# JuanJoZP/cfd-hemodynamic

Hardware: AMD Instinct MI355X
Metric: time-steps/sec, dfg_1 ~1M DOF (stabilized_schur) (higher is better)
Workload: dtype f64 (fp32 only in the AMG matrix values of the flexible preconditioner and in a read-only copy of the Krylov basis that Gram-Schmidt reads in solves of >= 20 iterations)

## Files before the change

### cfd_hemodynamic_amd/_lib.py

```python
from __future__ import annotations

import ctypes as C
import os
import subprocess

import numpy as np

_HERE = os.path.dirname(os.path.abspath(__file__))
_SO = os.path.join(_HERE, "libcfdh.so")
_LIB = None

dp = C.POINTER(C.c_double)
ip = C.POINTER(C.c_int32)
lp = C.POINTER(C.c_int64)


class Options(C.Structure):
    _fields_ = [
        ("snes_rtol", C.c_double), ("snes_atol", C.c_double), ("snes_stol", C.c_double), ("snes_max_it", C.c_int32),
        ("ksp_rtol", C.c_double), ("ksp_atol", C.c_double), ("ksp_max_it", C.c_int32), ("ksp_restart", C.c_int32),
        ("cheb_degree", C.c_int32), ("cheb_ratio", C.c_double), ("schur_full", C.c_int32),
        ("amg_smooth_degree", C.c_int32), ("amg_smooth_ratio", C.c_double), ("amg_theta", C.c_double),
        ("amg_max_coarse", C.c_int32), ("pc_refresh", C.c_int32), ("remove_p_mean", C.c_int32), ("verbose", C.c_int32),
        ("pc_type", C.c_int32), ("cc_smooth_degree", C.c_int32), ("ksp_guess", C.c_int32),
# ... 73 lines not shown
    L.cfdh_update_dirichlet.argtypes = [vp, C.c_int, C.c_int64, ip, dp]
    L.cfdh_set_state.argtypes = [vp, dp, dp, dp, dp]
    L.cfdh_get_solution.argtypes = [vp, dp, dp]
    L.cfdh_set_time_scheme.argtypes = [vp, C.c_double, C.c_double, C.c_double, C.c_double]
    L.cfdh_set_previous2.argtypes = [vp, dp]
    L.cfdh_get_previous2.argtypes = [vp, dp]
    L.cfdh_shift_history.argtypes = [vp]
    L.cfdh_wall_shear_stress.argtypes = [vp, dp]
    L.cfdh_set_boundary_terms.argtypes = [vp, C.c_int, C.c_int, C.c_double]
    L.cfdh_set_formulation.argtypes = [vp, C.c_int]
    L.cfdh_set_pressure_boundaries.argtypes = [vp, C.c_int, ip, dp, C.c_double]
    L.cfdh_set_pressure_boundaries_ex.argtypes = [vp, C.c_int, ip, dp, C.c_double, C.POINTER(C.c_uint8), dp]
    L.cfdh_get_residual.argtypes = [vp, dp, dp]
    L.cfdh_get_previous.argtypes = [vp, dp, dp]
    L.cfdh_advance.argtypes = [vp]
    L.cfdh_advance_field.argtypes = [vp, C.c_int]
    L.cfdh_assemble.argtypes = [vp, C.c_int]
    L.cfdh_get_csr.argtypes = [vp, lp, ip, ip, dp]
    L.cfdh_spmv.argtypes = [vp, dp, dp]
    L.cfdh_solve_step.argtypes = [vp, C.POINTER(Stats)]
    L.cfdh_functional.argtypes = [vp, C.c_int, C.c_int, dp]
    L.cfdh_set_halo.argtypes = [vp, C.c_int, ip, lp, ip, lp, ip]
    L.cfdh_set_global_pressure_space.argtypes = [vp, C.c_int64, C.c_int64, ip, dp, ip, C.c_int64, ip]
    L.cfdh_comm_unique_id.argtypes = [C.c_void_p]
    L.cfdh_comm_init.argtypes = [vp, C.c_void_p, C.c_int, C.c_int]
    L.cfdh_comm_set_callbacks.argtypes = [vp, ALLREDUCE_FN, EXCHANGE_FN, C.c_void_p, C.c_int, C.c_int]
    L.cfdh_profile_enable.argtypes = [vp, C.c_int]
    L.cfdh_profile_get.argtypes = [vp, C.c_int, dp, lp]
    L.cfdh_profile_reset.argtypes = [vp]
    L.cfdh_info.argtypes = [vp, C.c_int]
    L.cfdh_info.restype = C.c_int64
    L.cfdh_set_schur_pcd.argtypes = [vp, C.c_int, C.c_int, C.c_int]
    L.cfdh_set_ksp_forcing.argtypes = [vp, C.c_int, C.c_double, C.c_double, C.c_double, C.c_double, C.c_double]
    L.cfdh_get_newton_history.argtypes = [vp, ip, dp, dp, ip, dp]
    L.cfdh_get_pcd_operator.argtypes = [vp, lp, ip, ip, dp, dp]
    L.cfdh_apply_preconditioner.argtypes = [vp, dp, dp]
    L.cfdh_apply_operator.argtypes = [vp, dp, dp, dp]
    L.cfdh_get_amg_operator.argtypes = [vp, C.c_int, C.c_int, C.c_int, lp, lp, lp, ip, ip, dp]
    L.cfdh_get_amg_vectors.argtypes = [vp, C.c_int, C.c_int, C.c_int, lp, dp]
    L.cfdh_krylov_vec_op.argtypes = [vp, C.c_int, C.c_int, C.c_int, C.c_int, dp, dp, dp, dp, dp, C.c_double, C.c_int, dp, dp,
                                     C.POINTER(C.c_float), ip, dp, dp, dp]
    L.cfdh_create_ipcs.argtypes = [C.POINTER(vp), C.c_int, C.c_int, C.c_int64, C.c_int64, C.c_int64, ip, dp, C.c_int64, ip, ip, ip]
    L.cfdh_ipcs_set_form.argtypes = [vp, C.c_double, C.c_double]
    L.cfdh_ipcs_set_tolerances.argtypes = [vp, dp, C.c_double, ip]
    L.cfdh_ipcs_step.argtypes = [vp, C.POINTER(IpcsStats)]
    L.cfdh_ipcs_get_operator.argtypes = [vp, C.c_int, lp, ip, ip, dp]
    L.cfdh_ipcs_get_intermediate.argtypes = [vp, C.c_int, dp]
    L.cfdh_ipcs_apply_pressure_pc.argtypes = [vp, dp, dp]
    L.cfdh_ipcs_krylov_solve.argtypes = [vp, C.c_int, dp, dp, C.c_double, C.c_double, C.c_int, dp, C.POINTER(IpcsStats), dp]
    L.cfdh_wall_stats_reset.argtypes = [vp]
    L.cfdh_wall_stats_accumulate.argtypes = [vp, C.c_double]
    L.cfdh_wall_stats_get.argtypes = [vp, C.c_int, lp, dp]
    _LIB = L
    return L


def _dp(a):
    return None if a is None else a.ctypes.data_as(dp)


def _ip(a):
    return None if a is None else a.ctypes.data_as(ip)


def _lp(a):
    return None if a is None else a.ctypes.data_as(lp)


class CfdhError(RuntimeError):
    pass


def _raise(code, msg):
    if code == -1:
        raise ValueError(msg)
    raise CfdhError(msg)


FORM_CONVECTIVE, FORM_ROTATIONAL = 0, 1
PC_SELFP, PC_CAHOUET_CHABARD, PC_PCD = 0, 1, 2
AMG_HIER_A, AMG_HIER_P, AMG_HIER_H = 0, 1, 2
AMG_HIER_PG, AMG_HIER_DL0 = 3, 4
AMG_OP_A, AMG_OP_P, AMG_OP_G, AMG_OP_SB, AMG_OP_SC, AMG_OP_PT = 0, 1, 2, 3, 4, 5
(AMG_VEC_DINV, AMG_VEC_WDINV, AMG_VEC_AGG, AMG_VEC_COARSE_INV, AMG_VEC_D, AMG_VEC_LAMBDA, AMG_VEC_CC_SCALARS, AMG_VEC_CC_ML,
 AMG_VEC_CC_PBC, AMG_VEC_SPGEMM_ROWS, AMG_VEC_SHAPE, AMG_VEC_ORDER, AMG_VEC_A00_LMAX, AMG_VEC_A00_DINV, AMG_VEC_DL0_SHAPE) = range(15)
IP_RHO, IP_RHO_OLD, IP_ALPHA, IP_OMEGA, IP_BETA, IP_RZ, IP_TOL2, IP_BN2, IP_RN2, IP_DONE, IP_ITS, IP_BAD = range(12)
IP_NSCAL = 16

(KVOP_DOT, KVOP_NORM2, KVOP_NORM2_PAIR, KVOP_NORM2_TRIPLE, KVOP_NORMINF_DIFF, KVOP_SUB_MEAN, KVOP_NORM_SCALE_INV, KVOP_MULTIDOT,
 KVOP_MULTIDOT32, KVOP_GRAM, KVOP_MULTIAXPY, KVOP_LINCOMB, KVOP_LINCOMB_KEEP, KVOP_GS_UPDATE_NORMALIZE, KVOP_GS_UPDATE32, KVOP_STORE32,
 KVOP_GUESS, KVOP_AXPY, KVOP_WAXPY, KVOP_SCALE, KVOP_SCALE_TO, KVOP_PMULT) = range(22)
KVOP_FLAG_OPTION, KVOP_FLAG_RING = 1, 2
EW_DEFAULTS = (0.3, 0.9, 1.0, (1.0 + 5.0 ** 0.5) / 2.0, 0.1)
WALL_TAWSS, WALL_OSI, WALL_RRT, WALL_MEAN, WALL_PEAK, WALL_TOTALS = range(6)
INFO_WALL_STATS_COUNT = 90


class Context:

    def __init__(self, x, cells, facet_cells, facet_local, facet_marker, nv_owned=None, device=0, etype=0):
        L = lib()
        self.L = L
        x = np.asarray(x, dtype=np.float64)
        cells = np.asarray(cells)
        self.etype = int(etype)
        self.dim = (3 if x.shape[1] >= 3 and cells.shape[1] in (8, 10) or (self.etype == 3 and cells.shape[1] == 4) else 2) if self.etype \
            else cells.shape[1] - 1
        if self.dim not in (2, 3) or x.shape[1] < self.dim:
            raise ValueError("cells must be triangles [nc,3] or tetrahedra [nc,4] with matching coordinates")
        nodes = {(1, 2): 6, (2, 2): 4, (3, 2): 3, (1, 3): 10, (2, 3): 8, (3, 3): 4}
        if self.etype and cells.shape[1] != nodes[(self.etype, self.dim)]:
            raise ValueError("element type %d needs %d nodes per cell for gdim %d" % (self.etype, nodes[(self.etype, self.dim)], self.dim))
        self.x = np.ascontiguousarray(x[:, : self.dim]).copy()
        self.cells = np.ascontiguousarray(cells, dtype=np.int32)
        self.nv = len(self.x)
        self.nvo = self.nv if nv_owned is None else int(nv_owned)
        fc = np.ascontiguousarray(facet_cells, dtype=np.int32)
        fl = np.ascontiguousarray(facet_local, dtype=np.int32)
        fm = np.ascontiguousarray(facet_marker, dtype=np.int32)
        h = C.c_void_p()
        if self.etype:
            if self.nvo != self.nv:
                rc = L.cfdh_create_elem_part(C.byref(h), int(device), self.dim, self.etype, self.nv, self.nvo, len(self.cells), _ip(self.cells),
                                             _dp(self.x), len(fc), _ip(fc), _ip(fl), _ip(fm))
            else:
                rc = L.cfdh_create_elem(C.byref(h), int(device), self.dim, self.etype, self.nv, len(self.cells), _ip(self.cells), _dp(self.x),
                                        len(fc), _ip(fc), _ip(fl), _ip(fm))
        else:
            rc = L.cfdh_create(C.byref(h), int(device), self.dim, self.nv, self.nvo, len(self.cells), _ip(self.cells), _dp(self.x),
                               len(fc), _ip(fc), _ip(fl), _ip(fm))
        if rc != 0:
            _raise(rc, "cfdh_create failed: " + L.cfdh_last_error(None).decode())
        self.h = h
        self._cb = None

    def close(self):
        if getattr(self, "h", None):
            self.L.cfdh_destroy(self.h)
            self.h = None

    def __del__(self):
        try:
            self.close()
        except Exception:
            pass

    def _chk(self, rc):
        if rc != 0:
            _raise(rc, self.L.cfdh_last_error(self.h).decode())

    def set_params(self, dt, rho, mu, mu_facet=None, f=(0.0, 0.0)):
        ff = np.zeros(3)
        f = np.atleast_1d(np.asarray(f, dtype=np.float64))[:3]
        ff[: len(f)] = f
        self._chk(self.L.cfdh_set_params(self.h, dt, rho, mu, mu if mu_facet is None else mu_facet, _dp(ff)))

    def default_options(self):
        o = Options()
        self.L.cfdh_default_options(C.byref(o))
        return o

    def set_options(self, o):
        self._chk(self.L.cfdh_set_options(self.h, C.byref(o)))

    def clear_dirichlet(self):
        self._chk(self.L.cfdh_clear_dirichlet(self.h))
# ... 379 lines not shown
```

### cfd_hemodynamic_amd/csrc/cfdh_amg_apply.hip

```cpp
#include <hip/hip_runtime.h>

#include "cfdh_internal.hpp"
#include "cfdh_wave.hpp"

struct d3 { double x, y, z; };
__device__ __forceinline__ d3 vzero(const d3 *) { return d3{0.0, 0.0, 0.0}; }
__device__ __forceinline__ d3 vfma(double a, d3 x, d3 acc) { return d3{acc.x + a * x.x, acc.y + a * x.y, acc.z + a * x.z}; }
__device__ __forceinline__ d3 vsub(d3 a, d3 b) { return d3{a.x - b.x, a.y - b.y, a.z - b.z}; }
__device__ __forceinline__ d3 vadd(d3 a, d3 b) { return d3{a.x + b.x, a.y + b.y, a.z + b.z}; }
__device__ __forceinline__ d3 vscale(double a, d3 x) { return d3{a * x.x, a * x.y, a * x.z}; }
__device__ __forceinline__ d3 g8(d3 v) { return d3{group8_sum(v.x), group8_sum(v.y), group8_sum(v.z)}; }
__device__ __forceinline__ d3 wsum(d3 v) { return d3{wave_sum(v.x), wave_sum(v.y), wave_sum(v.z)}; }
__device__ __forceinline__ double vzero(const double *) { return 0.0; }
__device__ __forceinline__ double2 vzero(const double2 *) { return make_double2(0.0, 0.0); }
__device__ __forceinline__ double vfma(double a, double x, double acc) { return acc + a * x; }
__device__ __forceinline__ double2 vfma(double a, double2 x, double2 acc) { return make_double2(acc.x + a * x.x, acc.y + a * x.y); }
__device__ __forceinline__ double vsub(double a, double b) { return a - b; }
__device__ __forceinline__ double2 vsub(double2 a, double2 b) { return make_double2(a.x - b.x, a.y - b.y); }
__device__ __forceinline__ double vadd(double a, double b) { return a + b; }
__device__ __forceinline__ double2 vadd(double2 a, double2 b) { return make_double2(a.x + b.x, a.y + b.y); }
__device__ __forceinline__ double vscale(double a, double x) { return a * x; }
__device__ __forceinline__ double2 vscale(double a, double2 x) { return make_double2(a * x.x, a * x.y); }
__device__ __forceinline__ double g8(double v) { return group8_sum(v); }
__device__ __forceinline__ double2 g8(double2 v) { return make_double2(group8_sum(v.x), group8_sum(v.y)); }
__device__ __forceinline__ double wsum(double v) { return wave_sum(v); }
__device__ __forceinline__ double2 wsum(double2 v) { return make_double2(wave_sum(v.x), wave_sum(v.y)); }

template <int MAXW, typename T>
__device__ __forceinline__ T sell_row_dot(const int *__restrict__ sp, const int *__restrict__ sc, const float *__restrict__ sv,
                                          const T *__restrict__ x, int sl, int lane, T a) {
  sl = __builtin_amdgcn_readfirstlane(sl);
  const int p0 = sp[sl], w = (sp[sl + 1] - p0) >> 6;
  int cidx[MAXW];
  float cval[MAXW];
#pragma unroll
  for (int k = 0; k < MAXW; k++)
    if (k < w) { const int p = p0 + k * 64 + lane; cidx[k] = NTLOAD(sc + p); cval[k] = NTLOAD(sv + p); }
  T g[MAXW];
#pragma unroll
  for (int k = 0; k < MAXW; k++)
    if (k < w) g[k] = x[cidx[k]];
#pragma unroll
  for (int k = 0; k < MAXW; k++)
    if (k < w) a = vfma((double)cval[k], g[k], a);
  for (int k = MAXW; k < w; k++) { const int p = p0 + k * 64 + lane; a = vfma((double)sv[p], x[sc[p]], a); }
  return a;
}

template <int MODE, typename T>
__global__ __launch_bounds__(TPB) void csr_spmv_kernel(int n, const int *__restrict__ rowptr, const int *__restrict__ col,
                                                       const double *__restrict__ val, const T *__restrict__ x,
                                                       T *__restrict__ y, const T *__restrict__ b) {
  const int gid = blockIdx.x * TPB + threadIdx.x;
  const int row = gid >> 3, l = gid & 7;
  T a = vzero((const T *)nullptr);
  if (row < n) {
    const int ks = rowptr[row], ke = rowptr[row + 1];
    for (int k = ks + l; k < ke; k += 8) a = vfma(val[k], x[col[k]], a);
  }
  a = g8(a);
  if (row < n && l == 0) {
    if (MODE == 0) y[row] = a;
    else if (MODE == 1) y[row] = vsub(b[row], a);
    else if (MODE == 2) y[row] = vadd(y[row], a);
    else y[row] = vadd(b[row], a);
  }
}

template <typename T>
static int csr_spmv_t(cfdh_ctx *c, const CsrDev &A, const T *x, T *y, int mode, const T *b) {
  const long long nthreads = 8ll * A.n;
  dim3 grid((unsigned)((nthreads + TPB - 1) / TPB)), block(TPB);
  if (mode == 0) hipLaunchKernelGGL((csr_spmv_kernel<0, T>), grid, block, 0, c->stream, A.n, A.rowptr.p, A.col.p, A.val.p, x, y, b);
  else if (mode == 1) hipLaunchKernelGGL((csr_spmv_kernel<1, T>), grid, block, 0, c->stream, A.n, A.rowptr.p, A.col.p, A.val.p, x, y, b);
  else if (mode == 2) hipLaunchKernelGGL((csr_spmv_kernel<2, T>), grid, block, 0, c->stream, A.n, A.rowptr.p, A.col.p, A.val.p, x, y, b);
  else hipLaunchKernelGGL((csr_spmv_kernel<3, T>), grid, block, 0, c->stream, A.n, A.rowptr.p, A.col.p, A.val.p, x, y, b);
  HIPCHK(c, hipGetLastError());
  return 0;
}
int k_csr_spmv(cfdh_ctx *c, const CsrDev &A, const double *x, double *y, int mode, const double *b) {
  return csr_spmv_t<double>(c, A, x, y, mode, b);
}
int k_csr_spmv_ncol(cfdh_ctx *c, const CsrDev &A, const double *x, double *y, int mode, const double *b, int ncol) {
  if (ncol == 2) return csr_spmv_t<double2>(c, A, (const double2 *)x, (double2 *)y, mode, (const double2 *)b);
  if (ncol == 3) return csr_spmv_t<d3>(c, A, (const d3 *)x, (d3 *)y, mode, (const d3 *)b);
  return csr_spmv_t<double>(c, A, x, y, mode, b);
}

template <int MODE, bool LAST>
__global__ __launch_bounds__(TPB) void cheb_csr_step_kernel(int n, const int *__restrict__ rowptr, const int *__restrict__ col,
                                                            const double *__restrict__ val, const double *__restrict__ dinv,
                                                            const double *__restrict__ rin, double *__restrict__ rout,
                                                            const double *__restrict__ dold, double *__restrict__ dnew,
                                                            double *__restrict__ x, double c1, double c2, double itheta) {
  const int gid = blockIdx.x * TPB + threadIdx.x;
  const int row = gid >> 3, l = gid & 7;
  double a = 0;
  if (row < n) {
    const int ks = rowptr[row], ke = rowptr[row + 1];
    for (int k = ks + l; k < ke; k += 8) {
      const int j = col[k];
      a += val[k] * (MODE == 1 ? dinv[j] * rin[j] * itheta : dold[j]);
    }
  }
  a = group8_sum(a);
  if (row < n && l == 0) {
    const double di = dinv[row], ri = rin[row];
    const double dd = (MODE == 1) ? di * ri * itheta : dold[row];
    const double r = ri - a;
    const double dn = c1 * dd + c2 * di * r;
    if (!LAST) { rout[row] = r; dnew[row] = dn; }
    if (MODE == 0) x[row] += dn;
    else if (MODE == 1) x[row] = dd + dn;
    else x[row] += dd + dn;
  }
}

__global__ __launch_bounds__(TPB) void csr_resid_init_kernel(int n, const int *__restrict__ rowptr, const int *__restrict__ col,
                                                             const double *__restrict__ val, const double *__restrict__ dinv,
                                                             const double *__restrict__ b, const double *__restrict__ x,
                                                             double *__restrict__ r, double *__restrict__ d0, double itheta) {
  const int gid = blockIdx.x * TPB + threadIdx.x;
  const int row = gid >> 3, l = gid & 7;
  double a = 0;
  if (row < n) {
    const int ks = rowptr[row], ke = rowptr[row + 1];
    for (int k = ks + l; k < ke; k += 8) a += val[k] * x[col[k]];
  }
  a = group8_sum(a);
  if (row < n && l == 0) {
    const double rr = b[row] - a;
    r[row] = rr;
    d0[row] = dinv[row] * rr * itheta;
  }
}

static int level_cheb(cfdh_ctx *c, AmgLevel *L, const double *b, double *x, bool zero_guess, int deg, bool prof) {
  const int n = L->n;
  const double theta = 0.5 * (L->lmax + L->lmin), delta = 0.5 * (L->lmax - L->lmin), sigma = theta / delta;
  double rho = 1.0 / sigma;
  double *dold = L->d0.p, *dnew = L->d1.p, *r = L->r.p;
  const double *rin = b;
  const double itheta = 1.0 / theta;
  const long long nthreads = 8ll * n;
  dim3 grid((unsigned)((nthreads + TPB - 1) / TPB)), block(TPB);
  const int *rp = L->A.rowptr.p, *cl = L->A.col.p;
  const double *vl = L->A.val.p, *di = L->dinv.p;
  if (deg == 1) {
    if (!zero_guess) { CHK(k_csr_spmv(c, L->A, x, r, 1, b)); rin = r; }
    return k_cheb_init(c, n, di, rin, dold, x, itheta, zero_guess ? 0 : 1, nullptr);
  }
  if (!zero_guess) {
    hipLaunchKernelGGL(csr_resid_init_kernel, grid, block, 0, c->stream, n, rp, cl, vl, di, b, x, r, dold, itheta);
    rin = r;
  }
  for (int k = 1; k < deg; k++) {
    const double rho_new = 1.0 / (2.0 * sigma - rho);
    const double c1 = rho_new * rho, c2 = 2.0 * rho_new / delta;
    const bool last = (k == deg - 1);
    const int mode = (k == 1) ? (zero_guess ? 1 : 2) : 0;
    if (prof) prof_begin(c, 4);
#define LAUNCH_STEP(M, LST) hipLaunchKernelGGL((cheb_csr_step_kernel<M, LST>), grid, block, 0, c->stream, n, rp, cl, vl, di, rin, r, dold, dnew, x, c1, c2, itheta)
    if (mode == 1) { if (last) LAUNCH_STEP(1, true); else LAUNCH_STEP(1, false); }
    else if (mode == 2) { if (last) LAUNCH_STEP(2, true); else LAUNCH_STEP(2, false); }
    else { if (last) LAUNCH_STEP(0, true); else LAUNCH_STEP(0, false); }
#undef LAUNCH_STEP
    if (prof) prof_end(c, 4);
    rin = r;
    std::swap(dold, dnew);
    rho = rho_new;
  }
  HIPCHK(c, hipGetLastError());
  return 0;
}
int k_level_smooth(cfdh_ctx *c, AmgLevel *L, const double *b, double *x, int degree) { return level_cheb(c, L, b, x, true, degree, false); }

__global__ __launch_bounds__(TPB) void sell_cheb2_scale_kernel(int n, const int *__restrict__ sptr, const int *__restrict__ scol,
                                                               const float *__restrict__ svalw, const double *__restrict__ wdinv,
                                                               const double *__restrict__ dinv, const double *__restrict__ b,
                                                               double *__restrict__ x, const double *__restrict__ ml,
                                                               double *__restrict__ y, double c1, double c2) {
  const int row = blockIdx.x * TPB + threadIdx.x;
  if (row >= n) return;
  const int sl = row >> 6, lane = row & 63;
  const int p0 = sptr[sl], w = (sptr[sl + 1] - p0) >> 6;
  (void)p0; (void)w;
  const double a = sell_row_dot<10, double>(sptr, scol, svalw, b, sl, lane, 0.0);
  const double bi = b[row];
  const double dd = wdinv[row] * bi;
  const double xv = dd + (c1 * dd + c2 * dinv[row] * (bi - a));
  x[row] = xv;
  y[row] = ml[row] * xv;
}
bool k_cc_cheb2_scale(cfdh_ctx *c, AmgLevel *L, const double *b, double *x, const double *ml, double *y) {
  const int n = L->n;
  if (!(cfdh_cheb2_sell(L->A.nnz, n) && L->A.has_sell_weighted())) return false;
  const double theta = 0.5 * (L->lmax + L->lmin), delta = 0.5 * (L->lmax - L->lmin), sigma = theta / delta;
  const double rho = 1.0 / sigma, rho_new = 1.0 / (2.0 * sigma - rho);
  const double c1 = rho_new * rho, c2 = 2.0 * rho_new / delta;
  hipLaunchKernelGGL(sell_cheb2_scale_kernel, dim3((n + TPB - 1) / TPB), dim3(TPB), 0, c->stream, n, L->A.sptr.p, L->A.scol.p,
                     L->A.svalw.p, L->wdinv.p, L->dinv.p, b, x, ml, y, c1, c2);
  return hipGetLastError() == hipSuccess;
}

template <typename T>
__global__ __launch_bounds__(64) void dense_mv_kernel(int n, const double *__restrict__ Minv, const T *__restrict__ b,
                                                      T *__restrict__ y) {
  const int row = blockIdx.x, l = threadIdx.x;
  T a = vzero((const T *)nullptr);
  for (int k = l; k < n; k += 64) a = vfma(Minv[(size_t)row * n + k], b[k], a);
  a = wsum(a);
  if (l == 0) y[row] = a;
}

template <typename T>
__global__ __launch_bounds__(TPB) void jacobi_pre_kernel(int n, const int *__restrict__ rowptr, const int *__restrict__ col,
                                                         const double *__restrict__ val, const double *__restrict__ wdinv,
                                                         const T *__restrict__ b, T *__restrict__ xa, T *__restrict__ r) {
  const int gid = blockIdx.x * TPB + threadIdx.x;
  const int row = gid >> 3, l = gid & 7;
  T a = vzero((const T *)nullptr);
  if (row < n) {
    const int ks = rowptr[row], ke = rowptr[row + 1];
    for (int k = ks + l; k < ke; k += 8) {
      const int j = col[k];
      a = vfma(val[k] * wdinv[j], b[j], a);
    }
  }
  a = g8(a);
  if (row < n && l == 0) {
    const T bi = b[row];
    xa[row] = vscale(wdinv[row], bi);
    r[row] = vsub(bi, a);
  }
}
template <typename T>
__global__ __launch_bounds__(TPB) void jacobi_post_kernel(int n, const int *__restrict__ rowptr, const int *__restrict__ col,
                                                          const double *__restrict__ val, const double *__restrict__ wdinv,
                                                          const T *__restrict__ b, const T *__restrict__ xin,
                                                          T *__restrict__ xout) {
  const int gid = blockIdx.x * TPB + threadIdx.x;
  const int row = gid >> 3, l = gid & 7;
  T a = vzero((const T *)nullptr);
  if (row < n) {
    const int ks = rowptr[row], ke = rowptr[row + 1];
    for (int k = ks + l; k < ke; k += 8) a = vfma(val[k], xin[col[k]], a);
  }
  a = g8(a);
  if (row < n && l == 0) {
    xout[row] = vadd(xin[row], vscale(wdinv[row], vsub(b[row], a)));
  }
}

template <int MODE, typename T>
__global__ __launch_bounds__(TPB) void sell_spmv_kernel(int n, const int *__restrict__ sptr, const int *__restrict__ scol,
                                                        const float *__restrict__ sval, const T *__restrict__ x,
                                                        T *__restrict__ y, const T *__restrict__ b) {
  const int row = blockIdx.x * TPB + threadIdx.x;
  if (row >= n) return;
  const int sl = row >> 6, lane = row & 63;
  const int p0 = sptr[sl], w = (sptr[sl + 1] - p0) >> 6;
  T a = vzero((const T *)nullptr);
#pragma unroll 4
  for (int k = 0; k < w; k++) {
    const int p = p0 + k * 64 + lane;
    a = vfma((double)sval[p], x[scol[p]], a);
  }
  if (MODE == 0) y[row] = a;
  else if (MODE == 1) y[row] = vsub(b[row], a);
  else if (MODE == 2) y[row] = vadd(y[row], a);
  else y[row] = vadd(b[row], a);
}
template <typename T>
__global__ __launch_bounds__(TPB) void sell_jacobi_pre_kernel(int n, const int *__restrict__ sptr, const int *__restrict__ scol,
                                                              const float *__restrict__ svalw, const double *__restrict__ wdinv,
                                                              const T *__restrict__ b, T *__restrict__ xa, T *__restrict__ r) {
  const int row = blockIdx.x * TPB + threadIdx.x;
  if (row >= n) return;
  const int sl = row >> 6, lane = row & 63;
  const int p0 = sptr[sl], w = (sptr[sl + 1] - p0) >> 6;
  T a = vzero((const T *)nullptr);
#pragma unroll 4
  for (int k = 0; k < w; k++) {
    const int p = p0 + k * 64 + lane;
// ... 20 lines not shown
  }
  xout[row] = vadd(xin[row], vscale(wdinv[row], vsub(b[row], a)));
}

template <typename T>
static void launch_jacobi_pre(cfdh_ctx *c, const CsrDev &A, bool sell, int n, const double *wdinv, const T *b, T *xa, T *r) {
  dim3 block(TPB), gridS((unsigned)((n + TPB - 1) / TPB)), gridC((unsigned)((8ll * n + TPB - 1) / TPB));
  if (cfdh_pre_takes_sell(A, sell))
    hipLaunchKernelGGL((sell_jacobi_pre_kernel<T>), gridS, block, 0, c->stream, n, A.sptr.p, A.scol.p, A.svalw.p, wdinv, b, xa, r);
  else
    hipLaunchKernelGGL((jacobi_pre_kernel<T>), gridC, block, 0, c->stream, n, A.rowptr.p, A.col.p, A.val.p, wdinv, b, xa, r);
}
template <typename T>
static void launch_jacobi_post(cfdh_ctx *c, const CsrDev &A, bool sell, int n, const double *wdinv, const T *b, const T *x1, T *x) {
  dim3 block(TPB), gridS((unsigned)((n + TPB - 1) / TPB)), gridC((unsigned)((8ll * n + TPB - 1) / TPB));
  if (cfdh_post_takes_sell(A, sell))
    hipLaunchKernelGGL((sell_jacobi_post_kernel<T>), gridS, block, 0, c->stream, n, A.sptr.p, A.scol.p, A.sval.p, wdinv, b, x1, x);
  else
    hipLaunchKernelGGL((jacobi_post_kernel<T>), gridC, block, 0, c->stream, n, A.rowptr.p, A.col.p, A.val.p, wdinv, b, x1, x);
}
template <typename T>
static void launch_prolong_add(cfdh_ctx *c, const CsrDev &P, bool sell, int n, const T *x, T *y, const T *b) {
  dim3 block(TPB), gridS((unsigned)((n + TPB - 1) / TPB)), gridC((unsigned)((8ll * n + TPB - 1) / TPB));
  if (cfdh_prolong_takes_sell(P, sell))
    hipLaunchKernelGGL((sell_spmv_kernel<3, T>), gridS, block, 0, c->stream, n, P.sptr.p, P.scol.p, P.sval.p, x, y, b);
  else
    hipLaunchKernelGGL((csr_spmv_kernel<3, T>), gridC, block, 0, c->stream, n, P.rowptr.p, P.col.p, P.val.p, x, y, b);
}

template <typename T>
static int amg_cycle_jacobi(cfdh_ctx *c, AmgHier &H, size_t lev, const T *b, T *x, int prof) {
  AmgLevel *L = H.lev[lev];
  if (lev + 1 == H.lev.size()) {
    if (H.coarse_n > 0) {
      hipLaunchKernelGGL((dense_mv_kernel<T>), dim3(H.coarse_n), dim3(64), 0, c->stream, H.coarse_n, H.coarse_inv.p, b, x);
    } else {
      const int n = L->n;
      T *xa = (T *)L->d0.p, *r = (T *)L->r.p;
      launch_jacobi_pre<T>(c, L->A, false, n, L->wdinv.p, b, xa, r);
      launch_jacobi_post<T>(c, L->A, false, n, L->wdinv.p, b, (const T *)xa, x);
    }
    HIPCHK(c, hipGetLastError());
    return 0;
  }
  AmgLevel *N = H.lev[lev + 1];
  const int n = L->n;
  const bool sell = cfdh_sweep_sell(L->A.nnz, n);
  T *xa = (T *)L->d0.p, *x1 = (T *)L->d1.p, *r = (T *)L->r.p;
  if (prof && lev == 0) prof_begin(c, prof);
  launch_jacobi_pre<T>(c, L->A, sell, n, L->wdinv.p, b, xa, r);
  if (prof && lev == 0) prof_end(c, prof);
  CHK(csr_spmv_t<T>(c, L->R, r, (T *)N->b.p, 0, (const T *)nullptr));
  CHK(amg_cycle_jacobi<T>(c, H, lev + 1, (const T *)N->b.p, (T *)N->x.p, prof));
  launch_prolong_add<T>(c, L->P, sell, n, (const T *)N->x.p, x1, (const T *)xa);
  HIPCHK(c, hipGetLastError());
  if (prof && lev == 0) prof_begin(c, prof);
  launch_jacobi_post<T>(c, L->A, sell, n, L->wdinv.p, b, (const T *)x1, x);
  if (prof && lev == 0) prof_end(c, prof);
  HIPCHK(c, hipGetLastError());
  return 0;
}

template <int LPR>
__device__ __forceinline__ double lpr_sum(double v) {
  v = group8_sum(v);
  if (LPR >= 16) v += dpp_shuffle<0x140>(v);
  if (LPR >= 32) v += __shfl_xor(v, 16);
  if (LPR >= 64) v += __shfl_xor(v, 32);
  return v;
}
template <int LPR> __device__ __forceinline__ double lsum(double v) { return lpr_sum<LPR>(v); }
template <int LPR> __device__ __forceinline__ double2 lsum(double2 v) { return make_double2(lpr_sum<LPR>(v.x), lpr_sum<LPR>(v.y)); }
template <int LPR> __device__ __forceinline__ d3 lsum(d3 v) { return d3{lpr_sum<LPR>(v.x), lpr_sum<LPR>(v.y), lpr_sum<LPR>(v.z)}; }

__device__ __forceinline__ double epi_apply(double acc, int row, double alpha, double beta, const double *zH, const double *r, const unsigned char *pbc) {
  return (pbc[row] & 1) ? r[row] : alpha * acc + beta * zH[row];
}
__device__ __forceinline__ double2 epi_apply(double2 acc, int, double, double, const double *, const double *, const unsigned char *) { return acc; }
__device__ __forceinline__ double epi_value(double acc, unsigned flag, double alpha, double beta, double zh, double r) { return (flag & 1u) ? r : alpha * acc + beta * zh; }
__device__ __forceinline__ double2 epi_value(double2 acc, unsigned, double, double, double, double) { return acc; }
__device__ __forceinline__ d3 epi_apply(d3 acc, int, double, double, const double *, const double *, const unsigned char *) { return acc; }
__device__ __forceinline__ d3 epi_value(d3 acc, unsigned, double, double, double, double) { return acc; }

template <int LPR, typename VT, typename T>
__global__ __launch_bounds__(TPB) void fused_down_kernel(int n, const int *__restrict__ rowptr, const int *__restrict__ col,
                                                         const VT *__restrict__ val, const T *__restrict__ x, T *__restrict__ y) {
  const int gid = blockIdx.x * TPB + threadIdx.x;
  const int row = gid / LPR, l = gid % LPR;
  T a = vzero((const T *)nullptr);
  if (row < n) {
    const int ks = rowptr[row], ke = rowptr[row + 1];
    int cidx[4];
    VT cval[4];
#pragma unroll
    for (int q = 0; q < 4; q++) { const int k = ks + l + q * LPR; if (k < ke) { cidx[q] = col[k]; cval[q] = val[k]; } }
    T g[4];
#pragma unroll
    for (int q = 0; q < 4; q++) { const int k = ks + l + q * LPR; if (k < ke) g[q] = x[cidx[q]]; }
#pragma unroll
    for (int q = 0; q < 4; q++) { const int k = ks + l + q * LPR; if (k < ke) a = vfma((double)cval[q], g[q], a); }
    for (int k = ks + l + 4 * LPR; k < ke; k += LPR) a = vfma((double)val[k], x[col[k]], a);
  }
  a = lsum<LPR>(a);
  if (row < n && l == 0) y[row] = a;
}
template <typename T>
__global__ __launch_bounds__(TPB) void fused_up_csr_kernel(int n, const int *__restrict__ rpB, const int *__restrict__ clB,
                                                           const double *__restrict__ vlB, const T *__restrict__ b,
                                                           const int *__restrict__ rpC, const int *__restrict__ clC,
                                                           const double *__restrict__ vlC, const T *__restrict__ xc,
                                                           T *__restrict__ x, double ea, double eb, const double *__restrict__ ezH,
                                                           const double *__restrict__ er, const unsigned char *__restrict__ epbc) {
  const int gid = blockIdx.x * TPB + threadIdx.x;
  const int row = gid >> 3, l = gid & 7;
  T a = vzero((const T *)nullptr);
  if (row < n) {
    const int kb = rpB[row] + l, keB = rpB[row + 1];
    int kc = 0, keC = 0;
    if (rpC) { kc = rpC[row] + l; keC = rpC[row + 1]; }
    int cb[2], cc[2];
    double vb[2], vc[2];
#pragma unroll
    for (int q = 0; q < 2; q++) {
      if (kb + 8 * q < keB) { cb[q] = clB[kb + 8 * q]; vb[q] = vlB[kb + 8 * q]; }
      if (kc + 8 * q < keC) { cc[q] = clC[kc + 8 * q]; vc[q] = vlC[kc + 8 * q]; }
    }
    T gb[2], gc[2];
#pragma unroll
    for (int q = 0; q < 2; q++) {
      if (kb + 8 * q < keB) gb[q] = b[cb[q]];
      if (kc + 8 * q < keC) gc[q] = xc[cc[q]];
    }
#pragma unroll
    for (int q = 0; q < 2; q++) {
      if (kb + 8 * q < keB) a = vfma(vb[q], gb[q], a);
      if (kc + 8 * q < keC) a = vfma(vc[q], gc[q], a);
    }
    for (int k = kb + 16; k < keB; k += 8) a = vfma(vlB[k], b[clB[k]], a);
    for (int k = kc + 16; k < keC; k += 8) a = vfma(vlC[k], xc[clC[k]], a);
  }
  a = g8(a);
  if (row < n && l == 0) x[row] = epbc ? epi_apply(a, row, ea, eb, ezH, er, epbc) : a;
}
template <typename T, bool WIDE>
__global__ __launch_bounds__(TPB) void fused_up_sell_kernel(int n, const int *__restrict__ spB, const int *__restrict__ scB,
                                                            const float *__restrict__ svB, const T *__restrict__ b,
                                                            const int *__restrict__ spC, const int *__restrict__ scC,
                                                            const float *__restrict__ svC, const T *__restrict__ xc,
                                                            T *__restrict__ x, double ea, double eb, const double *__restrict__ ezH,
                                                            const double *__restrict__ er, const unsigned char *__restrict__ epbc) {
  const int row = blockIdx.x * TPB + threadIdx.x;
  if (row >= n) return;
  const int sl = __builtin_amdgcn_readfirstlane(row >> 6), lane = row & 63;
  T a = vzero((const T *)nullptr);
  double e_zh = 0.0, e_r = 0.0;
  unsigned e_f = 0;
  if (epbc) { e_f = epbc[row]; e_zh = ezH[row]; e_r = er[row]; }
  constexpr int MW = sizeof(T) > 8 ? 8 : 10;
  const int pB = spB[sl], wB = (spB[sl + 1] - pB) >> 6;
  int pC = 0, wC = 0;
  if (spC) { pC = spC[sl]; wC = (spC[sl + 1] - pC) >> 6; }
  const int wmax = wB > wC ? wB : wC;
  for (int k0 = 0; k0 < (WIDE ? wmax : 1); k0 += MW) {
    int cB[MW], cC[MW];
    float vB[MW], vC[MW];
#pragma unroll
    for (int k = 0; k < MW; k++) if (k0 + k < wB) { const int p = pB + (k0 + k) * 64 + lane; cB[k] = NTLOAD(scB + p); vB[k] = NTLOAD(svB + p); }
#pragma unroll
    for (int k = 0; k < MW; k++) if (k0 + k < wC) { const int p = pC + (k0 + k) * 64 + lane; cC[k] = NTLOAD(scC + p); vC[k] = NTLOAD(svC + p); }
    T gB[MW], gC[MW];
#pragma unroll
    for (int k = 0; k < MW; k++) if (k0 + k < wB) gB[k] = b[cB[k]];
#pragma unroll
    for (int k = 0; k < MW; k++) if (k0 + k < wC) gC[k] = xc[cC[k]];
#pragma unroll
    for (int k = 0; k < MW; k++) if (k0 + k < wB) a = vfma((double)vB[k], gB[k], a);
#pragma unroll
    for (int k = 0; k < MW; k++) if (k0 + k < wC) a = vfma((double)vC[k], gC[k], a);
  }
  if (!WIDE) {
    for (int k = MW; k < wB; k++) { const int p = pB + k * 64 + lane; a = vfma((double)svB[p], b[scB[p]], a); }
    for (int k = MW; k < wC; k++) { const int p = pC + k * 64 + lane; a = vfma((double)svC[p], xc[scC[p]], a); }
  }
  x[row] = epbc ? epi_value(a, e_f, ea, eb, e_zh, e_r) : a;
}
template <typename T>
__global__ __launch_bounds__(TPB) void fused_up_dense_kernel(int n, const int *__restrict__ rpB, const int *__restrict__ clB,
                                                             const double *__restrict__ vlB, const T *__restrict__ b,
                                                             const float *__restrict__ D, int nc, const T *__restrict__ bc,
                                                             T *__restrict__ x) {
  const int gid = blockIdx.x * TPB + threadIdx.x;
  const int row = gid >> 6, l = gid & 63;
  T a = vzero((const T *)nullptr);
  if (row < n) {
    for (int k = rpB[row] + l, ke = rpB[row + 1]; k < ke; k += 64) a = vfma(vlB[k], b[clB[k]], a);
    const float *Dr = D + (size_t)row * nc;
    float dv[12];
    T bv[12];
#pragma unroll
    for (int q = 0; q < 12; q++) { const int j = l + 64 * q; if (j < nc) { dv[q] = Dr[j]; bv[q] = bc[j]; } }
#pragma unroll
    for (int q = 0; q < 12; q++) { const int j = l + 64 * q; if (j < nc) a = vfma((double)dv[q], bv[q], a); }
    for (int j = l + 768; j < nc; j += 64) a = vfma((double)Dr[j], bc[j], a);
  }
  a = wsum(a);
  if (row < n && l == 0) x[row] = a;
}

template <typename VT, typename T>
static void launch_down(cfdh_ctx *c, const CsrDev &G, const VT *val, const T *x, T *y) {
  const long long avg = G.n > 0 ? (G.nnz + G.n - 1) / G.n : 1;
  const int lpr = avg > 96 ? 64 : (avg > 48 ? 32 : (avg > 20 ? 16 : 8));
  dim3 block(TPB), grid((unsigned)(((long long)G.n * lpr + TPB - 1) / TPB));
  if (lpr == 64) hipLaunchKernelGGL((fused_down_kernel<64, VT, T>), grid, block, 0, c->stream, G.n, G.rowptr.p, G.col.p, val, x, y);
  else if (lpr == 32) hipLaunchKernelGGL((fused_down_kernel<32, VT, T>), grid, block, 0, c->stream, G.n, G.rowptr.p, G.col.p, val, x, y);
  else if (lpr == 16) hipLaunchKernelGGL((fused_down_kernel<16, VT, T>), grid, block, 0, c->stream, G.n, G.rowptr.p, G.col.p, val, x, y);
  else hipLaunchKernelGGL((fused_down_kernel<8, VT, T>), grid, block, 0, c->stream, G.n, G.rowptr.p, G.col.p, val, x, y);
}

template <typename T>
static int amg_cycle_fused(cfdh_ctx *c, AmgHier &H, const T *b, T *x, int prof, int l0 = 0) {
  const int nl = (int)H.lev.size();
  for (int l = l0; l + 1 < nl; l++) {
    AmgLevel *L = H.lev[l], *N = H.lev[l + 1];
    const T *src = l == l0 ? b : (const T *)L->b.p;
    if (prof && l == 0) prof_begin(c, prof + 4);
    if (L->fine) launch_down<float, T>(c, L->G, L->G.valf.p, src, (T *)N->b.p);
    else launch_down<double, T>(c, L->G, L->G.val.p, src, (T *)N->b.p);
    if (prof && l == 0) prof_end(c, prof + 4);
  }
  int l = nl - 1;
  {
    AmgLevel *L = H.lev[l];
    const T *bl = l == l0 ? b : (const T *)L->b.p;
    T *xl = l == l0 ? x : (T *)L->x.p;
    if (nl - 2 >= l0 && H.lev[nl - 2]->Dn > 0) {
      AmgLevel *U = H.lev[nl - 2];
      const T *bu = nl - 2 == l0 ? b : (const T *)U->b.p;
      T *xu = nl - 2 == l0 ? x : (T *)U->x.p;
      const int un = (nl - 2 == 0 && c->up0_rows > 0 && c->up0_rows < U->n) ? c->up0_rows : U->n;
      hipLaunchKernelGGL((fused_up_dense_kernel<T>), dim3((unsigned)((64ll * un + TPB - 1) / TPB)), dim3(TPB), 0, c->stream, un,
                         U->Sb.rowptr.p, U->Sb.col.p, U->Sb.val.p, bu, U->D.p, U->Dn, bl, xu);
      l = nl - 3;
    } else {
      if (H.coarse_n > 0)
        hipLaunchKernelGGL((dense_mv_kernel<T>), dim3(H.coarse_n), dim3(64), 0, c->stream, H.coarse_n, H.coarse_inv.p, bl, xl);
      else if (L->sell)
        hipLaunchKernelGGL((fused_up_sell_kernel<T, true>), dim3((unsigned)((L->n + TPB - 1) / TPB)), dim3(TPB), 0, c->stream, L->n,
                           L->Sb.sptr.p, L->Sb.scol.p, L->Sb.sval.p, bl, (const int *)nullptr, (const int *)nullptr,
                           (const float *)nullptr, (const T *)nullptr, xl, 0.0, 0.0, (const double *)nullptr, (const double *)nullptr,
                           (const unsigned char *)nullptr);
      else
        hipLaunchKernelGGL((fused_up_csr_kernel<T>), dim3((unsigned)((8ll * L->n + TPB - 1) / TPB)), dim3(TPB), 0, c->stream, L->n,
                           L->Sb.rowptr.p, L->Sb.col.p, L->Sb.val.p, bl, (const int *)nullptr, (const int *)nullptr,
                           (const double *)nullptr, (const T *)nullptr, xl, 0.0, 0.0, (const double *)nullptr, (const double *)nullptr,
                           (const unsigned char *)nullptr);
      l = nl - 2;
    }
  }
  for (; l >= l0; l--) {
    AmgLevel *L = H.lev[l], *N = H.lev[l + 1];
    const T *bl = l == l0 ? b : (const T *)L->b.p;
    T *xl = l == l0 ? x : (T *)L->x.p;
    const bool epi = l == 0 && c->epi.on && sizeof(T) == sizeof(double);
    const double ea = epi ? c->epi.alpha : 0.0, eb = epi ? c->epi.beta : 0.0;
    const double *ezH = epi ? c->epi.zH : nullptr, *er = epi ? c->epi.r : nullptr;
    const unsigned char *epbc = epi ? c->epi.pbc : nullptr;
    if (epi) { xl = (T *)c->epi.out; c->epi.done = true; }
    const int nrow = (l == 0 && c->up0_rows > 0 && c->up0_rows < L->n) ? c->up0_rows : L->n;
    if (prof && l == 0) prof_begin(c, prof);
    if (L->sell && L->Sb.sell_maxw <= 14 && L->Sc.sell_maxw <= 14)
      hipLaunchKernelGGL((fused_up_sell_kernel<T, false>), dim3((unsigned)((nrow + TPB - 1) / TPB)), dim3(TPB), 0, c->stream, nrow,
                         L->Sb.sptr.p, L->Sb.scol.p, L->Sb.sval.p, bl, L->Sc.sptr.p, L->Sc.scol.p, L->Sc.sval.p, (const T *)N->x.p, xl,
                         ea, eb, ezH, er, epbc);
    else if (L->sell)
      hipLaunchKernelGGL((fused_up_sell_kernel<T, true>), dim3((unsigned)((nrow + TPB - 1) / TPB)), dim3(TPB), 0, c->stream, nrow,
                         L->Sb.sptr.p, L->Sb.scol.p, L->Sb.sval.p, bl, L->Sc.sptr.p, L->Sc.scol.p, L->Sc.sval.p, (const T *)N->x.p, xl,
                         ea, eb, ezH, er, epbc);
    else
      hipLaunchKernelGGL((fused_up_csr_kernel<T>), dim3((unsigned)((8ll * nrow + TPB - 1) / TPB)), dim3(TPB), 0, c->stream, nrow,
                         L->Sb.rowptr.p, L->Sb.col.p, L->Sb.val.p, bl, L->Sc.rowptr.p, L->Sc.col.p, L->Sc.val.p, (const T *)N->x.p, xl,
                         ea, eb, ezH, er, epbc);
    if (prof && l == 0) prof_end(c, prof);
  }
  HIPCHK(c, hipGetLastError());
  return 0;
}

static int amg_cycle_cheb(cfdh_ctx *c, AmgHier &H, size_t lev, const double *b, double *x, bool prof) {
  AmgLevel *L = H.lev[lev];
  if (lev + 1 == H.lev.size()) {
    if (H.coarse_n > 0) {
      hipLaunchKernelGGL((dense_mv_kernel<double>), dim3(H.coarse_n), dim3(64), 0, c->stream, H.coarse_n, H.coarse_inv.p, b, x);
      HIPCHK(c, hipGetLastError());
      return 0;
    }
    return level_cheb(c, L, b, x, true, c->opt.amg_smooth_degree > 2 ? c->opt.amg_smooth_degree : 2, false);
  }
  AmgLevel *N = H.lev[lev + 1];
  const int deg = c->opt.amg_smooth_degree;
  CHK(level_cheb(c, L, b, x, true, deg, prof && lev == 0));
  CHK(k_csr_spmv(c, L->A, x, L->r.p, 1, b));
  CHK(k_csr_spmv(c, L->R, L->r.p, N->b.p, 0, nullptr));
  CHK(amg_cycle_cheb(c, H, lev + 1, N->b.p, N->x.p, prof));
  CHK(k_csr_spmv(c, L->P, N->x.p, x, 2, nullptr));
  CHK(level_cheb(c, L, b, x, false, deg, prof && lev == 0));
  return 0;
}

__global__ __launch_bounds__(TPB) void dl0_pack_kernel(int nvo, int nv, int dim, const double *__restrict__ vec, const double *__restrict__ wdinv,
                                                       double *__restrict__ b, double *__restrict__ xa, int ghosts) {
  const int i = blockIdx.x * TPB + threadIdx.x;
  if (i >= nv) return;
  const double v = i < nvo ? vec[(size_t)dim * nvo + i] : (ghosts ? vec[((size_t)dim + 1) * nvo + ((size_t)dim + 1) * (size_t)(i - nvo) + dim] : 0.0);
  b[i] = v;
  xa[i] = wdinv[i] * v;
}
int k_dl0_down(cfdh_ctx *c, const double *halo_vec) {
  cfdh_ctx::DistL0 &d = c->dl0;
  AmgLevel *N = c->hLg.lev[1];
  const int nvo = c->nvo, nv = c->nv;
  if (d.ghost_rhs) hipLaunchKernelGGL(dl0_pack_kernel, dim3((nv + TPB - 1) / TPB), dim3(TPB), 0, c->stream, nvo, nv, c->dim, halo_vec, d.wdinv.p, d.b.p, d.xa.p, 1);
  launch_jacobi_pre<double>(c, d.A, cfdh_dl0_rule_A(c), nvo, d.wdinv.p, (const double *)d.b.p, d.xa.p, d.r.p);
  HIPCHK(c, hipGetLastError());
  return csr_spmv_t<double>(c, d.PT, d.r.p, N->b.p, 0, (const double *)nullptr);
}
int k_dl0_up(cfdh_ctx *c, double *out) {
  cfdh_ctx::DistL0 &d = c->dl0;
  AmgLevel *N = c->hLg.lev[1];
  const int nvo = c->nvo, nv = c->nv;
  if (cfdh_dl0_coarse_fused(c)) CHK(amg_cycle_fused<double>(c, c->hLg, (const double *)N->b.p, N->x.p, 0, 1));
  else CHK(amg_cycle_jacobi<double>(c, c->hLg, 1, (const double *)N->b.p, N->x.p, 0));
  launch_prolong_add<double>(c, d.P, cfdh_dl0_rule_P(c), nv, (const double *)N->x.p, d.x1.p, (const double *)d.xa.p);
  HIPCHK(c, hipGetLastError());
  launch_jacobi_post<double>(c, d.A, cfdh_dl0_rule_A(c), nvo, d.wdinv.p, (const double *)d.b.p, (const double *)d.x1.p, out);
  HIPCHK(c, hipGetLastError());
  return 0;
}

int k_amg_vcycle(cfdh_ctx *c, AmgHier &H, const double *b, double *x) {
  if (!H.valid || H.lev.empty()) return cfdh_fail(c, CFDH_E_STATE, "AMG hierarchy not built");
  const bool prof = (&H == &c->hS) || (&H == &c->hL) || (&H == &c->hLg);
  if (H.ncol == 3) {
    if (H.fused && c->opt.amg_smooth_degree == 1 && H.lev.size() >= 2) return amg_cycle_fused<d3>(c, H, (const d3 *)b, (d3 *)x, 5);
    return amg_cycle_jacobi<d3>(c, H, 0, (const d3 *)b, (d3 *)x, 5);
  }
  if (H.fused && c->opt.amg_smooth_degree == 1 && H.lev.size() >= 2) {
    if (H.ncol == 2) return amg_cycle_fused<double2>(c, H, (const double2 *)b, (double2 *)x, 5);
    return amg_cycle_fused<double>(c, H, b, x, prof ? 4 : 0);
  }
  if (H.ncol == 2) return amg_cycle_jacobi<double2>(c, H, 0, (const double2 *)b, (double2 *)x, 5);
  if (c->opt.amg_smooth_degree == 1) return amg_cycle_jacobi<double>(c, H, 0, b, x, prof ? 4 : 0);
  return amg_cycle_cheb(c, H, 0, b, x, prof);
}

__global__ __launch_bounds__(TPB) void cc_scale_kernel(int n, const double *__restrict__ ml, const double *__restrict__ z, double *__restrict__ y) {
  const int i = blockIdx.x * TPB + threadIdx.x;
  if (i < n) y[i] = ml[i] * z[i];
}
__global__ __launch_bounds__(TPB) void cc_combine_kernel(int n, double alpha, double beta, const double *__restrict__ t,
                                                         const double *__restrict__ z, const double *__restrict__ r,
                                                         const unsigned char *__restrict__ pbc, double *__restrict__ out, double *__restrict__ out2) {
  const int i = blockIdx.x * TPB + threadIdx.x;
  if (i < n) {
    const double v = (pbc[i] & 1) ? r[i] : alpha * t[i] + beta * z[i];
// ... 59 lines not shown
```

### cfd_hemodynamic_amd/csrc/cfdh_api.cpp

```cpp
#include <algorithm>
#include <cmath>
#include <numeric>

#include <dlfcn.h>

#include "cfdh_internal.hpp"
#include "cfdh_ipcs.hpp"

std::string g_cfdh_last_error;

int cfdh_prepare_assembly(cfdh_ctx *c);

#define ENTER(c)                         \
  do {                                   \
    if (!(c)) return CFDH_E_ARG;         \
    (void)hipSetDevice((c)->device);     \
  } while (0)

#define NOT_IPCS(c, name)                                                                                                    \
  do {                                                                                                                       \
    if ((c) && (c)->ipcs) return cfdh_fail((c), CFDH_E_STATE, name ": not available on an incremental pressure-correction context (cfdh_create_ipcs)"); \
  } while (0)
#define NEED_IPCS(c, name)                                                                                         \
  do {                                                                                                             \
    if (!(c)) return CFDH_E_ARG;                                                                                   \
    if (!(c)->ipcs) return cfdh_fail((c), CFDH_E_STATE, name ": the context was not created by cfdh_create_ipcs"); \
    (void)hipSetDevice((c)->device);                                                                               \
  } while (0)

static int ipcs_put(cfdh_ctx *c, dbuf<double> &dst, const double *src) {
  if (!src) return 0;
  c->ipcs->n_field_copies++;
  HIPCHK(c, hipMemcpyAsync(dst.p, src, sizeof(double) * dst.n, hipMemcpyHostToDevice, c->stream));
  HIPCHK(c, hipStreamSynchronize(c->stream));
  return 0;
}
static int ipcs_get(cfdh_ctx *c, const dbuf<double> &src, double *dst) {
  if (!dst) return 0;
  c->ipcs->n_field_copies++;
  HIPCHK(c, hipMemcpyAsync(dst, src.p, sizeof(double) * src.n, hipMemcpyDeviceToHost, c->stream));
  HIPCHK(c, hipStreamSynchronize(c->stream));
  return 0;
}
static int ipcs_copy(cfdh_ctx *c, const dbuf<double> &src, dbuf<double> &dst) {
  HIPCHK(c, hipMemcpyAsync(dst.p, src.p, sizeof(double) * src.n, hipMemcpyDeviceToDevice, c->stream));
  return 0;
}

namespace {
template <class T>
struct HookBuf {
  T *p = nullptr;
  ~HookBuf() { if (p) (void)hipFree(p); }
  int put(cfdh_ctx *c, const T *src, size_t count, size_t filled) {
    HIPCHK(c, hipMalloc((void **)&p, sizeof(T) * count));
    HIPCHK(c, hipMemsetAsync(p, 0, sizeof(T) * count, c->stream));
    if (src && filled) HIPCHK(c, hipMemcpyAsync(p, src, sizeof(T) * filled, hipMemcpyHostToDevice, c->stream));
    return 0;
  }
  int get(cfdh_ctx *c, T *dst, size_t count) const {
    HIPCHK(c, hipMemcpy(dst, p, sizeof(T) * count, hipMemcpyDeviceToHost));
    return 0;
  }
};
}

extern "C" {

int cfdh_abi_version(void) { return CFDH_ABI_VERSION; }

const char *cfdh_last_error(const cfdh_ctx *c) { return c ? c->err.c_str() : g_cfdh_last_error.c_str(); }

int cfdh_default_options(cfdh_options *o) {
  if (!o) return CFDH_E_ARG;
  o->snes_rtol = 1e-8; o->snes_atol = 1e-50; o->snes_stol = 1e-8; o->snes_max_it = 100;
  o->ksp_rtol = 1e-5; o->ksp_atol = 1e-50; o->ksp_max_it = 1000; o->ksp_restart = 200;
  o->cheb_degree = 3; o->cheb_ratio = 10.0; o->schur_full = 2;
  o->amg_smooth_degree = 1; o->amg_smooth_ratio = 8.0; o->amg_theta = -1.0; o->amg_max_coarse = 1000;
  o->pc_refresh = 0; o->remove_p_mean = 1; o->verbose = 0; o->pc_type = 1; o->cc_smooth_degree = 2;
  o->ksp_guess = getenv("CFDH_KSP_GUESS") ? atoi(getenv("CFDH_KSP_GUESS")) : 4;
  return 0;
}

static int create_ctx(cfdh_ctx **out, int device, int gdim, int etype, int64_t nv, int64_t nv_owned, int64_t nc, const int32_t *cells,
                      const double *coords, int64_t nfacets, const int32_t *facet_cells, const int32_t *facet_local,
                      const int32_t *facet_marker) {
  if (!out) return cfdh_fail(nullptr, CFDH_E_ARG, "null output pointer");
  *out = nullptr;
  if (gdim != 2 && gdim != 3) return cfdh_fail(nullptr, CFDH_E_ARG, "gdim must be 2 (P1 triangles) or 3 (P1 tetrahedra)");
  if (etype < 0 || etype > 3) return cfdh_fail(nullptr, CFDH_E_ARG, "unknown element type %d", etype);
  if (!cells || !coords || (nfacets > 0 && (!facet_cells || !facet_local)))
    return cfdh_fail(nullptr, CFDH_E_ARG, "null mesh array");
  int ndev = 0;
  if (hipGetDeviceCount(&ndev) != hipSuccess || ndev <= 0)
    return cfdh_fail(nullptr, CFDH_E_HIP, "no HIP device available: libcfdh has no CPU fallback");
  if (device < 0 || device >= ndev) return cfdh_fail(nullptr, CFDH_E_ARG, "device %d out of range (%d devices)", device, ndev);
  cfdh_ctx *c = new (std::nothrow) cfdh_ctx();
  if (!c) return cfdh_fail(nullptr, CFDH_E_NOMEM, "out of host memory");
  c->device = device;
  cfdh_default_options(&c->opt);
  { const char *e = getenv("CFDH_NO_GRAPH"); c->use_graph = !(e && e[0] == '1'); }
  { const char *e = getenv("CFDH_SOLVE_LEAN"); c->lean = !(e && e[0] == '0'); }
  {
    cfdh_ctx::SolveEnv &v = c->env;
    const char *e;
    if ((e = getenv("CFDH_KRYLOV_FP32"))) v.krylov_fp32 = atoi(e);
    v.guess_check = getenv("CFDH_GUESS_CHECK") != nullptr;
    e = getenv("CFDH_NO_ATTAINABLE_STOP"); v.no_attainable_stop = e && e[0] == '1';
    if ((e = getenv("CFDH_GS_REFINE_FROM"))) v.gs_refine_from = atoi(e);
    if ((e = getenv("CFDH_KSP_LAG"))) v.ksp_lag = atoi(e);
    if ((e = getenv("CFDH_GS_ETA2"))) v.gs_eta2 = atof(e);
    if ((e = getenv("CFDH_L_CYCLES"))) v.l_cycles = atoi(e);
    if ((e = getenv("CFDH_A_CYCLES"))) v.a_cycles = atoi(e);
    e = getenv("CFDH_DL0_COARSE_SWEEPS"); v.dl0_coarse_sweeps = e && e[0] == '1';
  }
  if (c->use_graph && (getenv("ROCP_TOOL_LIBRARIES") || dlsym(RTLD_DEFAULT, "rocprofiler_configure"))) {
    int rt = 0;
    const char *ov = getenv("CFDH_GRAPH_UNDER_PROFILER");
    if (!(ov && ov[0] == '1') && hipRuntimeGetVersion(&rt) == hipSuccess && rt >= 70200000) c->use_graph = false;
  }
  memset(&c->last_stats, 0, sizeof c->last_stats);
  int rc = 0;
  do {
    if (hipSetDevice(device) != hipSuccess) { rc = cfdh_fail(nullptr, CFDH_E_HIP, "hipSetDevice(%d) failed", device); break; }
    if (hipStreamCreateWithFlags(&c->stream, hipStreamNonBlocking) != hipSuccess) { rc = cfdh_fail(nullptr, CFDH_E_HIP, "hipStreamCreate failed"); break; }
    rc = gdim == 3 ? k3_upload_quadrature(c) : k_upload_quadrature(c);
    if (rc) break;
    if (etype != 0) {
      rc = gdim == 3 ? kg3_upload_tables(c) : kg_upload_tables(c);
      if (rc) break;
      rc = gdim == 3 ? cfdh_build_mesh_gen3(c, etype, nv, nv_owned, nc, cells, coords, nfacets, facet_cells, facet_local, facet_marker)
                     : cfdh_build_mesh_gen(c, etype, nv, nv_owned, nc, cells, coords, nfacets, facet_cells, facet_local, facet_marker);
      break;
    }
    rc = gdim == 3 ? cfdh_build_mesh3(c, nv, nv_owned, nc, cells, coords, nfacets, facet_cells, facet_local, facet_marker)
                   : cfdh_build_mesh(c, nv, nv_owned, nc, cells, coords, nfacets, facet_cells, facet_local, facet_marker);
  } while (0);
  if (rc) {
    g_cfdh_last_error = c->err.empty() ? g_cfdh_last_error : c->err;
    cfdh_destroy(c);
    return rc;
  }
  *out = c;
  return 0;
}

int cfdh_create(cfdh_ctx **out, int device, int gdim, int64_t nv, int64_t nv_owned, int64_t nc, const int32_t *cells,
                const double *coords, int64_t nfacets, const int32_t *facet_cells, const int32_t *facet_local,
                const int32_t *facet_marker) {
  return create_ctx(out, device, gdim, CFDH_ELEM_P1, nv, nv_owned, nc, cells, coords, nfacets, facet_cells, facet_local, facet_marker);
}

int cfdh_create_elem(cfdh_ctx **out, int device, int gdim, int elem, int64_t nn, int64_t nc, const int32_t *cells, const double *node_coords,
                     int64_t nfacets, const int32_t *facet_cells, const int32_t *facet_local, const int32_t *facet_marker) {
  return create_ctx(out, device, gdim, elem, nn, nn, nc, cells, node_coords, nfacets, facet_cells, facet_local, facet_marker);
}

int cfdh_create_elem_part(cfdh_ctx **out, int device, int gdim, int elem, int64_t nn, int64_t nn_owned, int64_t nc, const int32_t *cells,
                          const double *node_coords, int64_t nfacets, const int32_t *facet_cells, const int32_t *facet_local, const int32_t *facet_marker) {
  return create_ctx(out, device, gdim, elem, nn, nn_owned, nc, cells, node_coords, nfacets, facet_cells, facet_local, facet_marker);
}

void cfdh_destroy(cfdh_ctx *c) {
  if (!c) return;
  (void)hipSetDevice(c->device);
  if (c->stream) (void)hipStreamSynchronize(c->stream);
  cfdh_ipcs_free(c);
  comm_finalize(c);
  c->hS.clear(); c->hL.clear(); c->hA.clear(); c->hLg.clear();
  for (hipEvent_t e : c->ev_pool) (void)hipEventDestroy(e);
  for (auto &e : c->pc_graphs) for (auto &x : e.exec) if (x) (void)hipGraphExecDestroy(x);
  if (c->h_pinned) (void)hipHostFree(c->h_pinned);
  if (c->h_stage) (void)hipHostFree(c->h_stage);
  if (c->ev_h) (void)hipEventDestroy(c->ev_h);
  if (c->h_big) (void)hipHostFree(c->h_big);
  if (c->h_ring) (void)hipHostFree(c->h_ring);
  for (hipEvent_t e : c->ev_ring) if (e) (void)hipEventDestroy(e);
  hipStream_t s = c->stream;
  delete c;
  if (s) (void)hipStreamDestroy(s);
}

int cfdh_set_params(cfdh_ctx *c, double dt, double rho, double mu, double mu_facet, const double f[3]) {
  ENTER(c);
  if (!(dt > 0) || !(rho > 0) || !(mu > 0)) return cfdh_fail(c, CFDH_E_ARG, "dt, rho, mu must be positive");
// ... 586 lines not shown
      CHK(v_multidot(c, n, dA.p, ld, nvec, dx.p, ds.p, ww, mir_dev)); nd = nm = nvec + (ww ? 1 : 0); break;
    }
    case CFDH_KVOP_MULTIDOT32: CHK(v_multidot32(c, n, dA32.p, ld, nvec, dx.p, ds.p, mir_dev)); nd = nm = nvec + 1; break;
    case CFDH_KVOP_GRAM: CHK(v_gram(c, n, dA.p, ld, nvec, dx.p, ds.p)); nd = 8 * (nvec + 1); break;
    case CFDH_KVOP_MULTIAXPY:
      HIPCHK(c, hipMemcpyAsync(d1.p, dx.p, sizeof(double) * N, hipMemcpyDeviceToDevice, c->stream));
      CHK(v_multiaxpy(c, n, dA.p, ld, nvec, dc.p, d1.p)); break;
    case CFDH_KVOP_LINCOMB:
      HIPCHK(c, hipMemcpyAsync(d1.p, dx.p, sizeof(double) * N, hipMemcpyDeviceToDevice, c->stream));
      CHK(v_lincomb(c, n, dA.p, ld, nvec, dc.p, d1.p)); break;
    case CFDH_KVOP_LINCOMB_KEEP:
      HIPCHK(c, hipMemcpyAsync(d1.p, dx.p, sizeof(double) * N, hipMemcpyDeviceToDevice, c->stream));
      CHK(v_lincomb_keep(c, n, dA.p, ld, nvec, dc.p, d1.p, d2.p)); break;
    case CFDH_KVOP_GS_UPDATE_NORMALIZE: CHK(v_gs_update_normalize(c, n, dA.p, ld, nvec, dc.p, dx.p, d1.p, ds.p)); nd = 1; break;
    case CFDH_KVOP_GS_UPDATE32:
      CHK(v_gs_update32(c, n, dA32.p, ld, nvec, dc.p, dx.p, d1.p, d32.p, ds.p, mir_dev + (nvec + 1))); nd = 1; nm = nvec + 2; break;
    case CFDH_KVOP_STORE32: CHK(v_store32(c, n, dx.p, d32.p)); break;
    case CFDH_KVOP_GUESS: {
      CHK(v_guess_combine(c, n, dA.p, dB.p, ld, nvec, dc.p, dx.p, d1.p, d2.p));
      bool used = false; int rank = 0;
      CHK(v_guess_read(c, nvec, scal_host, &used, &rank, scal_host + 3));
      scal_host[1] = used ? 1.0 : 0.0; scal_host[2] = (double)rank;
      if (flags & 1) CHK(v_scale_inv_lean(c, n, d2.p));
      ns = nm = 3 + nvec;
      HIPCHK(c, hipMemcpyAsync(ds.p, c->red_out.p + RO_LEAN_S2, sizeof(double), hipMemcpyDeviceToDevice, c->stream));
      HIPCHK(c, hipMemcpyAsync(ds.p + 1, c->ky.p, sizeof(double) * nvec, hipMemcpyDeviceToDevice, c->stream));
      nd = 1 + nvec; break;
    }
    case CFDH_KVOP_AXPY:
      HIPCHK(c, hipMemcpyAsync(d1.p, dy.p, sizeof(double) * N, hipMemcpyDeviceToDevice, c->stream));
      CHK(v_axpy(c, n, scalar, dx.p, d1.p)); break;
    case CFDH_KVOP_WAXPY: CHK(v_waxpy(c, n, scalar, dx.p, dy.p, d1.p)); break;
    case CFDH_KVOP_SCALE:
      HIPCHK(c, hipMemcpyAsync(d1.p, dx.p, sizeof(double) * N, hipMemcpyDeviceToDevice, c->stream));
      CHK(v_scale(c, n, scalar, d1.p)); break;
    case CFDH_KVOP_SCALE_TO: CHK(v_scale_to(c, n, scalar, dx.p, d1.p)); break;
    case CFDH_KVOP_PMULT: CHK(v_pointwise_mult(c, n, dx.p, dy.p, d1.p)); break;
  }
  HIPCHK(c, hipStreamSynchronize(c->stream));
  if (nd) HIPCHK(c, hipMemcpy(scal_dev, dev_src, sizeof(double) * nd, hipMemcpyDeviceToHost));
  for (int i = 0; i < nm; i++) scal_mirror[i] = mir_host[i];
  nscal[0] = ns; nscal[1] = nd; nscal[2] = nm;
  if (o1) CHK(d1.get(c, out1, N));
  if (o2) CHK(d2.get(c, out2, N));
  if (o32) CHK(d32.get(c, out32, N));
  return 0;
}

static int amg_pick(cfdh_ctx *c, const char *name, int hier, int level, AmgHier **H, AmgLevel **L) {
  if (!c->pc_valid) return cfdh_fail(c, CFDH_E_STATE, "%s: no preconditioner built yet (cfdh_apply_preconditioner or cfdh_solve_step first)", name);
  *H = nullptr;
  *L = nullptr;
  if (hier == CFDH_AMG_HIER_H) {
    if (c->opt.pc_type != 1 || c->Hlev.n <= 0) return cfdh_fail(c, CFDH_E_STATE, "%s: H exists for pc_type 1 only", name);
    *L = &c->Hlev;
    return 0;
  }
  if (hier == CFDH_AMG_HIER_DL0) {
    if (c->gp_n <= 0 || !c->hLg.valid || !c->dl0.on) return cfdh_fail(c, CFDH_E_STATE, "%s: no distributed finest pressure level on this context", name);
    *H = &c->hLg;
    return 0;
  }
  if (hier != CFDH_AMG_HIER_A && hier != CFDH_AMG_HIER_P && hier != CFDH_AMG_HIER_PG) return cfdh_fail(c, CFDH_E_ARG, "%s: unknown hierarchy %d", name, hier);
  if (hier == CFDH_AMG_HIER_A && c->opt.pc_type == 0) return cfdh_fail(c, CFDH_E_STATE, "%s: pc_type 0 has no velocity hierarchy", name);
  if (hier == CFDH_AMG_HIER_PG && c->gp_n <= 0) return cfdh_fail(c, CFDH_E_STATE, "%s: no replicated pressure space (cfdh_set_global_pressure_space)", name);
  AmgHier *h = hier == CFDH_AMG_HIER_A ? &c->hA : hier == CFDH_AMG_HIER_PG ? &c->hLg : (c->opt.pc_type == 0 ? &c->hS : &c->hL);
  if (!h->valid) return cfdh_fail(c, CFDH_E_STATE, "%s: hierarchy %d is not built", name, hier);
  if (level < 0 || level >= (int)h->lev.size()) return cfdh_fail(c, CFDH_E_ARG, "%s: level %d of %d", name, level, (int)h->lev.size());
  *H = h;
  *L = h->lev[level];
  return 0;
}
static bool amg_local_dim(const cfdh_ctx *c, int n) { return n == (int)c->perm.size() || n == c->nvo; }

int cfdh_get_amg_operator(cfdh_ctx *c, int hier, int level, int which, int64_t *nrow, int64_t *ncol, int64_t *nnz, int32_t *rowptr,
                          int32_t *col, double *vals) {
  NOT_IPCS(c, "cfdh_get_amg_operator");
  if (!c || !nrow || !ncol || !nnz) return CFDH_E_ARG;
  ENTER(c);
  AmgHier *H = nullptr;
  AmgLevel *L = nullptr;
  CHK(amg_pick(c, "cfdh_get_amg_operator", hier, level, &H, &L));
  const bool dl0 = hier == CFDH_AMG_HIER_DL0;
  if (dl0 ? (which != CFDH_AMG_OP_A && which != CFDH_AMG_OP_P && which != CFDH_AMG_OP_PT) : (which < CFDH_AMG_OP_A || which > CFDH_AMG_OP_SC))
    return cfdh_fail(c, CFDH_E_ARG, "cfdh_get_amg_operator: unknown operator %d", which);
  if (!H || dl0) level = 0;
  const CsrDev &M = dl0 ? (which == CFDH_AMG_OP_A ? c->dl0.A : which == CFDH_AMG_OP_P ? c->dl0.P : c->dl0.PT)
                        : which == CFDH_AMG_OP_A ? L->A : which == CFDH_AMG_OP_P ? L->P : which == CFDH_AMG_OP_G ? L->G : which == CFDH_AMG_OP_SB ? L->Sb : L->Sc;
  if (M.n <= 0 || !M.rowptr.p || !M.col.p || !M.val.p)
    return cfdh_fail(c, CFDH_E_STATE, "cfdh_get_amg_operator: operator %d of level %d is not kept in fp64 CSR (P: CFDH_AMG_KEEP=1 before the build)", which, level);
  *nrow = M.n; *ncol = M.m; *nnz = M.nnz;
  if (!rowptr && !col && !vals) return 0;
  if (!rowptr || !col || !vals) return cfdh_fail(c, CFDH_E_ARG, "pass all of rowptr/col/vals or none");
  std::vector<int> rp((size_t)M.n + 1), cl((size_t)M.nnz);
  std::vector<double> vl((size_t)M.nnz);
  HIPCHK(c, hipMemcpyAsync(rp.data(), M.rowptr.p, sizeof(int) * rp.size(), hipMemcpyDeviceToHost, c->stream));
  if (M.nnz > 0) {
    HIPCHK(c, hipMemcpyAsync(cl.data(), M.col.p, sizeof(int) * cl.size(), hipMemcpyDeviceToHost, c->stream));
    HIPCHK(c, hipMemcpyAsync(vl.data(), M.val.p, sizeof(double) * vl.size(), hipMemcpyDeviceToHost, c->stream));
  }
  HIPCHK(c, hipStreamSynchronize(c->stream));
  if (rp[M.n] != M.nnz) return cfdh_fail(c, CFDH_E_STATE, "cfdh_get_amg_operator: rowptr ends at %d, the operator holds %d entries", rp[M.n], M.nnz);
  const bool local0 = level == 0 && hier != CFDH_AMG_HIER_PG;
  const bool rows0 = local0 && which != CFDH_AMG_OP_G && which != CFDH_AMG_OP_PT && amg_local_dim(c, M.n);
  const bool cols0 = local0 && (which == CFDH_AMG_OP_A || which == CFDH_AMG_OP_SB || which == CFDH_AMG_OP_G || which == CFDH_AMG_OP_PT) && amg_local_dim(c, M.m);
  const bool resort = cols0 && which != CFDH_AMG_OP_PT;
  int64_t pos = 0;
  std::vector<std::pair<int, double>> row;
  for (int ru = 0; ru < M.n; ru++) {
    const int r = rows0 ? c->perm[ru] : ru;
    rowptr[ru] = (int32_t)pos;
    row.clear();
    for (int k = rp[r]; k < rp[r + 1]; k++) row.push_back({cols0 ? c->iperm[cl[k]] : cl[k], vl[k]});
    if (resort) std::stable_sort(row.begin(), row.end(), [](const std::pair<int, double> &a, const std::pair<int, double> &b) { return a.first < b.first; });
    for (auto &e : row) { col[pos] = e.first; vals[pos] = e.second; pos++; }
  }
  rowptr[M.n] = (int32_t)pos;
  return 0;
}

int cfdh_get_amg_vectors(cfdh_ctx *c, int hier, int level, int which, int64_t *n, double *out) {
  NOT_IPCS(c, "cfdh_get_amg_vectors");
  if (!c || !n) return CFDH_E_ARG;
  ENTER(c);
  AmgHier *H = nullptr;
  AmgLevel *L = nullptr;
  CHK(amg_pick(c, "cfdh_get_amg_vectors", hier, level, &H, &L));
  const bool dl0 = hier == CFDH_AMG_HIER_DL0;
  if (!H || dl0) level = 0;
  if (dl0 && which != CFDH_AMG_VEC_WDINV && which != CFDH_AMG_VEC_ORDER && which != CFDH_AMG_VEC_DL0_SHAPE)
    return cfdh_fail(c, CFDH_E_ARG, "cfdh_get_amg_vectors: the distributed level has no item %d", which);
  AmgLevel dl0_view;
  if (dl0) { dl0_view.n = c->nv; L = &dl0_view; }
  const bool perm0 = level == 0 && hier != CFDH_AMG_HIER_PG && amg_local_dim(c, L->n);
  auto fetch = [&](const void *src, size_t bytes, void *dst) -> int {
    HIPCHK(c, hipMemcpyAsync(dst, src, bytes, hipMemcpyDeviceToHost, c->stream));
    HIPCHK(c, hipStreamSynchronize(c->stream));
    return 0;
  };
  const int nvo = c->nvo;
  switch (which) {
    case CFDH_AMG_VEC_DINV:
    case CFDH_AMG_VEC_WDINV: {
      const dbuf<double> &v = dl0 ? c->dl0.wdinv : which == CFDH_AMG_VEC_DINV ? L->dinv : L->wdinv;
      if (!v.p || (int)v.n < L->n) return cfdh_fail(c, CFDH_E_STATE, "cfdh_get_amg_vectors: vector %d is not there", which);
      *n = L->n;
      if (!out) return 0;
      std::vector<double> h((size_t)L->n);
      CHK(fetch(v.p, sizeof(double) * h.size(), h.data()));
      for (int i = 0; i < L->n; i++) out[i] = h[perm0 ? c->perm[i] : i];
      return 0;
    }
    case CFDH_AMG_VEC_AGG: {
      if (!L->agg.p || (int)L->agg.n < L->n) return cfdh_fail(c, CFDH_E_STATE, "cfdh_get_amg_vectors: the aggregate ids were not kept (CFDH_AMG_KEEP=1 before the build)");
      *n = L->n;
      if (!out) return 0;
      std::vector<int> h((size_t)L->n);
      CHK(fetch(L->agg.p, sizeof(int) * h.size(), h.data()));
      for (int i = 0; i < L->n; i++) out[i] = (double)h[perm0 ? c->perm[i] : i];
      return 0;
    }
    case CFDH_AMG_VEC_COARSE_INV: {
      if (!H || H->coarse_n <= 0 || !H->coarse_inv.p) return cfdh_fail(c, CFDH_E_STATE, "cfdh_get_amg_vectors: no dense coarsest inverse");
      *n = (int64_t)H->coarse_n * H->coarse_n;
      if (!out) return 0;
      if (H->lev.size() == 1 && hier != CFDH_AMG_HIER_PG && amg_local_dim(c, H->coarse_n)) {
        const size_t m = (size_t)H->coarse_n;
        std::vector<double> h(m * m);
        CHK(fetch(H->coarse_inv.p, sizeof(double) * h.size(), h.data()));
        for (size_t i = 0; i < m; i++)
          for (size_t j = 0; j < m; j++) out[i * m + j] = h[(size_t)c->perm[i] * m + (size_t)c->perm[j]];
        return 0;
      }
      return fetch(H->coarse_inv.p, sizeof(double) * (size_t)*n, out);
    }
    case CFDH_AMG_VEC_D: {
      if (L->Dn <= 0 || !L->D.p) return cfdh_fail(c, CFDH_E_STATE, "cfdh_get_amg_vectors: level %d has no folded dense correction", level);
      *n = (int64_t)L->n * L->Dn;
      if (!out) return 0;
      std::vector<float> h((size_t)*n);
      CHK(fetch(L->D.p, sizeof(float) * h.size(), h.data()));
      for (int i = 0; i < L->n; i++) {
        const size_t r = (size_t)(perm0 ? c->perm[i] : i);
        for (int j = 0; j < L->Dn; j++) out[(size_t)i * L->Dn + j] = (double)h[r * L->Dn + j];
      }
// ... 471 lines not shown
  c->n_cycles = c->n_guess_projections = c->n_iter_sync = 0;
  c->n_krylov_discarded = 0;
  return 0;
}

int64_t cfdh_info(const cfdh_ctx *c, int what) {
  if (!c) return -1;
  if (c->ipcs) {
    const IpcsData *I = c->ipcs;
    switch (what) {
      case 0: case 1: return I->nn;
      case 2: return I->nc;
      case 3: return (int64_t)I->hM.col.size();
      case 6: return (int64_t)I->hLam.lev.size();
      case 15: return I->last.host_syncs;
      case 18: return 1;
      case 26: return I->D;
      case 29: return I->NL;
      case 80: return I->last.launches;
      case 81: return I->nvert;
      case 82: return I->n_field_copies;
      case 83: return 1;
      case 84: case 90: return c->ws_count;
      default: return -1;
    }
  }
  switch (what) {
    case 0: return c->nvo;
    case 1: return c->nv;
    case 2: return c->nc;
    case 3: return c->nnzv;
    case 4: return c->opt.pc_type >= 1 ? c->hL.fine_nnz : c->hS.fine_nnz;
    case 5: return c->ninc;
    case 6: return (int64_t)(c->opt.pc_type >= 1 ? c->hL.lev.size() : c->hS.lev.size());
    case 7: return c->nblk;
    case 8: return c->hA.fine_nnz;
    case 9: return c->gp_allgather ? c->gp_maxcnt : 0;
    case 10: return c->nccl_comm ? 1 : 0;
    case 11: return c->dl0.on ? c->dl0.n1 : 0;
    case 12: return c->ras ? 1 : 0;
    case 13: return c->n_allreduce;
    case 14: return c->n_halo;
    case 15: return c->n_host_sync;
    case 16: return c->n_krylov;
    case 17: return c->n_allgather;
    case 18: return c->nranks;
    case 26: return c->dim;
    case 30: case 31: case 32: case 33: case 34: case 35: case 36: case 37: case 38: case 39:
    case 40: case 41: case 42: case 43: case 44: case 45: case 46: case 47: case 48: case 49:
    case 50: case 51: case 52: case 53: case 54: case 55: case 56: case 57: case 58: case 59:
    case 60: case 61: case 62: case 63: case 64: case 65: case 66: case 67: case 68: case 69: {
      const AmgHier &h = what < 50 ? c->hA : (c->opt.pc_type >= 1 ? c->hL : c->hS);
      const size_t l = (size_t)(what % 10);
      if (l >= h.lev.size()) return 0;
      return ((what / 10) & 1) ? (int64_t)h.lev[l]->n : (int64_t)h.lev[l]->A.nnz;
    }
    case 28: return c->etype;
    case 70: return c->n_guess_solves;
    case 71: return c->n_guess_solves ? (int64_t)(1e6 * c->guess_reduction_sum / (double)c->n_guess_solves) : 0;
    case 29: return c->nloc;
    case 73: return c->n_krylov_discarded;
    case 74: return c->n_pc_builds;
    case 84: return c->n_cycles;
    case 86: return c->n_guess_projections;
    case 87: return c->n_iter_sync;
    case 88: return c->guess_last_rank;
    case 89: return c->guess_last_k;
    case 85: return c->lean ? 1 : 0;
    case 90: return c->ws_count;
    case 75: return c->pc_valid ? 1 : 0;
    case 76: return c->singular;
    case 77: return c->form;
    case 78: return c->opt.pc_type;
    case 79: return c->ew_version;
    case 72: return c->n_attainable_stops;
    case 27: return (int64_t)(1000.0 * c->ms_pc_build_dev);
    case 19: return c->opt.pc_type >= 1 ? c->hL.nnz_S0 : c->hS.nnz_S0;
    case 20: return c->hA.nnz_S0;
    case 21: return c->opt.pc_type >= 1 ? c->hL.nnz_G0 : c->hS.nnz_G0;
    case 22: return c->hA.nnz_G0;
    case 23: { const AmgHier &h = c->opt.pc_type >= 1 ? c->hL : c->hS; return h.lev.size() > 1 ? h.lev[1]->n : 0; }
    case 24: return c->hA.lev.size() > 1 ? c->hA.lev[1]->n : 0;
    case 25: { const AmgHier &h = c->opt.pc_type >= 1 ? c->hL : c->hS; return h.fused ? 1 : 0; }
    default: return -1;
  }
}


int cfdh_create_ipcs(cfdh_ctx **out, int device, int gdim, int64_t nn, int64_t nvert, int64_t nc, const int32_t *cells, const double *node_coords,
                     int64_t nfacets, const int32_t *facet_cells, const int32_t *facet_local, const int32_t *facet_marker) {
  if (!out) return cfdh_fail(nullptr, CFDH_E_ARG, "null output pointer");
  *out = nullptr;
  if (gdim != 2 && gdim != 3) return cfdh_fail(nullptr, CFDH_E_ARG, "gdim must be 2 (P2/P1 triangles) or 3 (P2/P1 tetrahedra)");
  if (!cells || !node_coords || nfacets < 0 || (nfacets > 0 && (!facet_cells || !facet_local))) return cfdh_fail(nullptr, CFDH_E_ARG, "null mesh array");
  int ndev = 0;
  if (hipGetDeviceCount(&ndev) != hipSuccess || ndev <= 0)
    return cfdh_fail(nullptr, CFDH_E_HIP, "no HIP device available: libcfdh has no CPU fallback");
  if (device < 0 || device >= ndev) return cfdh_fail(nullptr, CFDH_E_ARG, "device %d out of range (%d devices)", device, ndev);
  cfdh_ctx *c = new (std::nothrow) cfdh_ctx();
  if (!c) return cfdh_fail(nullptr, CFDH_E_NOMEM, "out of host memory");
  c->device = device;
  cfdh_default_options(&c->opt);
  c->use_graph = false;
  memset(&c->last_stats, 0, sizeof c->last_stats);
  int rc = 0;
  if (hipSetDevice(device) != hipSuccess) rc = cfdh_fail(nullptr, CFDH_E_HIP, "hipSetDevice(%d) failed", device);
  else if (hipStreamCreateWithFlags(&c->stream, hipStreamNonBlocking) != hipSuccess) rc = cfdh_fail(nullptr, CFDH_E_HIP, "hipStreamCreate failed");
  else rc = cfdh_ipcs_create(c, gdim, nn, nvert, nc, cells, node_coords, nfacets, facet_cells, facet_local, facet_marker);
  if (rc) {
    g_cfdh_last_error = c->err.empty() ? g_cfdh_last_error : c->err;
    cfdh_destroy(c);
    return rc;
  }
  *out = c;
  return 0;
}

int cfdh_ipcs_set_form(cfdh_ctx *c, double conv_coeff, double force_coeff) {
  NEED_IPCS(c, "cfdh_ipcs_set_form");
  if (!(conv_coeff >= 0) || !std::isfinite(conv_coeff) || !std::isfinite(force_coeff)) return cfdh_fail(c, CFDH_E_ARG, "cfdh_ipcs_set_form: conv_coeff >= 0 and finite coefficients");
  c->ipcs->conv_coeff = conv_coeff; c->ipcs->force_coeff = force_coeff; c->ipcs->force_default = false;
  c->ipcs->assembled = false;
  return 0;
}

int cfdh_ipcs_set_tolerances(cfdh_ctx *c, const double rtol[3], double atol, const int32_t max_it[3]) {
  NEED_IPCS(c, "cfdh_ipcs_set_tolerances");
  if (!rtol || !max_it || !(atol >= 0)) return cfdh_fail(c, CFDH_E_ARG, "cfdh_ipcs_set_tolerances: bad arguments");
  for (int k = 0; k < 3; k++)
    if (!(rtol[k] >= 0) || !(rtol[k] < 1) || max_it[k] < 1) return cfdh_fail(c, CFDH_E_ARG, "cfdh_ipcs_set_tolerances: 0 <= rtol < 1, max_it >= 1");
  for (int k = 0; k < 3; k++) { c->ipcs->rtol[k] = rtol[k]; c->ipcs->max_it[k] = max_it[k]; }
  c->ipcs->atol = atol;
  return 0;
}

int cfdh_ipcs_step(cfdh_ctx *c, cfdh_ipcs_stats *stats) {
  NEED_IPCS(c, "cfdh_ipcs_step");
  c->err.clear();
  cfdh_ipcs_stats st;
  const int rc = cfdh_ipcs_step_impl(c, &st);
  if (stats) *stats = st;
  return rc;
}

int cfdh_ipcs_get_operator(cfdh_ctx *c, int which, int64_t *nnz, int32_t *rowptr, int32_t *col, double *vals) {
  NEED_IPCS(c, "cfdh_ipcs_get_operator");
  IpcsData *I = c->ipcs;
  const int D = I->D;
  if (!nnz || which < 0 || which >= 3 + 2 * D) return cfdh_fail(c, CFDH_E_ARG, "cfdh_ipcs_get_operator: which in [0, %d)", 3 + 2 * D);
  const std::vector<int> &ptr = which == 1 ? I->hL.rowptr : which < 3 ? I->hM.rowptr : which < 3 + D ? I->bptr : I->gptr;
  const std::vector<int> &cl = which == 1 ? I->hL.col : which < 3 ? I->hM.col : which < 3 + D ? I->bcol : I->gcol;
  *nnz = (int64_t)cl.size();
  if (!rowptr && !col && !vals) return 0;
  if (!rowptr || !col || !vals) return cfdh_fail(c, CFDH_E_ARG, "pass all of rowptr/col/vals or none");
  std::copy(ptr.begin(), ptr.end(), rowptr);
  std::copy(cl.begin(), cl.end(), col);
  if (which >= 3) {
    const std::vector<double> &v = which < 3 + D ? I->hB : I->hG;
    const int d = which < 3 + D ? which - 3 : which - 3 - D;
    for (size_t k = 0; k < cl.size(); k++) vals[k] = v[(size_t)D * k + d];
    return 0;
  }
  if (which == 0) {
    if (!I->assembled) CHK(cfdh_ipcs_assemble(c));
  } else {
    if (!c->params_set) return cfdh_fail(c, CFDH_E_STATE, "cfdh_set_params was not called");
// ... 39 lines not shown
```

### cfd_hemodynamic_amd/csrc/cfdh_internal.hpp

```cpp
#pragma once
#include <hip/hip_runtime.h>

#include <cstdint>
#include <cstdio>
#include <cstring>
#include <string>
#include <vector>

#include "cfdh.h"
#include "cfdh_scratch.hpp"

#ifndef CFDH_MAX_INC
#define CFDH_MAX_INC 256
#endif
#ifndef CFDH_MAX_BV
#define CFDH_MAX_BV 192
#endif
#ifndef CFDH_MAX_BC
#define CFDH_MAX_BC 192
#endif
#ifndef CFDH_MAX_ROWS
#define CFDH_MAX_ROWS 128
#endif

#if defined(__HIPCC__)
__device__ __forceinline__ double cfdh_rsqrt(double x) {
  double y = __builtin_amdgcn_rsq(x);
  const double h = 0.5 * x;
  y = __builtin_fma(y, __builtin_fma(-h * y, y, 0.5), y);
  y = __builtin_fma(y, __builtin_fma(-h * y, y, 0.5), y);
  return y;
}
#endif

template <class T>
struct dbuf {
  T *p = nullptr;
  size_t n = 0;
  dbuf() = default;
  dbuf(const dbuf &) = delete;
  dbuf &operator=(const dbuf &) = delete;
  ~dbuf() { release(); }
  void release() {
    if (p) (void)hipFree(p);
    p = nullptr;
    n = 0;
  }
  hipError_t alloc(size_t count) {
    if (count == n && p) return hipSuccess;
    release();
    if (count == 0) return hipSuccess;
    hipError_t e = hipMalloc((void **)&p, count * sizeof(T));
    if (e == hipSuccess) n = count;
    return e;
  }
  hipError_t upload(const std::vector<T> &h, hipStream_t s) {
    hipError_t e = alloc(h.size());
    if (e != hipSuccess || h.empty()) return e;
    return hipMemcpyAsync(p, h.data(), h.size() * sizeof(T), hipMemcpyHostToDevice, s);
  }
  hipError_t zero(hipStream_t s) { return n ? hipMemsetAsync(p, 0, n * sizeof(T), s) : hipSuccess; }
  void adopt(dbuf &o) {
    if (&o == this) return;
    release();
    p = o.p; n = o.n;
    o.p = nullptr; o.n = 0;
  }
};

struct CsrHost {
  int n = 0, m = 0;
  std::vector<int> rowptr, col;
  std::vector<double> val;
  int nnz() const { return (int)col.size(); }
};

struct CsrDev {
  int n = 0, m = 0, nnz = 0;
  dbuf<int> rowptr, col;
  dbuf<double> val;
  int nslice = 0, sell_maxw = 0;
  dbuf<int> sptr, scol;
  dbuf<float> sval, svalw;
  dbuf<float> valf;
  bool has_sell() const { return sptr.p && scol.p && sval.p; }
  bool has_sell_weighted() const { return sptr.p && scol.p && svalw.p; }
};
enum { CFDH_UP_CSR = 1, CFDH_UP_SELL = 2, CFDH_UP_CSRF = 4};

inline bool cfdh_short_rows(long long nnz, int n, int per_row) { return nnz <= (long long)per_row * n && n >= 16384; }
inline bool cfdh_level_fine(int dim, long long nnz, int n) { return cfdh_short_rows(nnz, n, dim == 3 ? 20 : 12); }
inline bool cfdh_level_sell(int dim, long long nnz, int n, int ncol) {
  return cfdh_level_fine(dim, nnz, n) && (cfdh_short_rows(nnz, n, 12) || ncol == 1);
}
inline bool cfdh_sweep_sell(long long nnz, int n) { return cfdh_short_rows(nnz, n, 12); }
inline bool cfdh_cheb2_sell(long long nnz, int n) { return cfdh_short_rows(nnz, n, 20); }

struct AmgLevel {
  int n = 0;
  CsrDev A, P, R;
  dbuf<double> dinv, wdinv, x, b, r, d0, d1;
  double lmax = 0, lmin = 0;
  CsrDev G, Sb, Sc;
  dbuf<float> D;
  int Dn = 0;
  bool fine = false;
  bool sell = false;
  dbuf<int> agg;
};

struct AmgHier {
  std::vector<AmgLevel *> lev;
  dbuf<double> coarse_inv;
  int coarse_n = 0, ncol = 1;
  long long fine_nnz = 0;
  bool valid = false;
  bool fused = false;
  long long nnz_G0 = 0, nnz_S0 = 0;
  long long spgemm_rows[3] = {0, 0, 0};
  bool keep_host0 = false;
  CsrHost h_A0, h_P0;
  std::vector<double> h_wdinv0;
  void clear() {
    for (AmgLevel *l : lev) delete l;
    lev.clear();
    valid = false;
  }
  ~AmgHier() { clear(); }
};

struct ProfSlot {
  double total_ms = 0;
  long long launches = 0;
};

struct IpcsData;

struct cfdh_ctx {
  int device = 0;
  IpcsData *ipcs = nullptr;
  hipStream_t stream = nullptr;
  std::string err;

  int dim = 2;
  int etype = 0, nloc = 3;
  bool gen = false;
  dbuf<int> gslot;
  dbuf<int> g_eptr, g_fptr, g_fdst;
  dbuf<double> gE, gEF;
  dbuf<unsigned short> gflag;
  dbuf<unsigned char> gpbidx;
  dbuf<int> g3_fcells;
  int g3_nfcells = 0;
  dbuf<unsigned char> g3_pbslot;
  dbuf<int> g3_pcells;
  int g3_npcells = 0;
  CsrHost gen_P1;
  int nv = 0, nvo = 0, ng = 0, nc = 0, nfac = 0;
  int NL = 0;
  int NO = 0;

  std::vector<int> perm;
  std::vector<int> iperm;
  std::vector<int> h_cells;
  std::vector<int> cell_user;
  std::vector<double> h_coords;
  std::vector<int> fac_cell, fac_local, fac_marker;
  std::vector<int> fac_user;
  int nfac_user = 0;

  bool params_set = false;
  double dt = 0, rho = 0, mu = 0, muf = 0, f[3] = {0, 0, 0};
  cfdh_options opt;
// ... 113 lines not shown
  long long bc_version = 0;
  int gp_n = 0;
  CsrHost gp_L;
  bool gp_singular = false, gp_dirty = false;
  AmgHier hLg;
  dbuf<int> gp_l2g;
  dbuf<double> gp_rhs, gp_sol;
  bool ras = false;
  std::vector<int> h_gid;
  std::vector<int> h_g2l;
  dbuf<double> ras_b, ras_x;
  struct RasPlan {
    bool ready = false;
    int maxlen = 0;
    int nent = 0;
    dbuf<int> gptr, gcol, gsrc;
    dbuf<double> gval;
  } rasp;
  struct DistL0 {
    bool on = false;
    bool ghost_rhs = true;
    int n1 = 0;
    CsrDev A;
    CsrDev P;
    CsrDev PT;
    dbuf<double> wdinv, b, xa, r, x1;
  } dl0;
  bool gp_allgather = false;
  int gp_maxcnt = 0;
  dbuf<int> gp_send_idx;
  dbuf<int> gp_src_idx;
  dbuf<double> gp_sendbuf, gp_recvbuf;
  dbuf<double> pcw;
  double *h_big = nullptr;
  size_t h_big_n = 0;
  std::vector<unsigned char> hL_pbc;
  int hL_singular = -1;
  bool pc_valid = false;
  int pc_its_ref = 0;
  int steps_since_refresh = 0;
  int singular = 0;

  int nnbr = 0;
  std::vector<int> nbr_rank;
  std::vector<long long> send_ptr, recv_ptr;
  dbuf<int> send_idx;
  dbuf<double> send_buf;
  std::vector<double> h_send, h_recv;
  int rank = 0, nranks = 1;
  double nvo_global = 0;
  void *nccl_comm = nullptr;
  cfdh_allreduce_fn cb_ar = nullptr;
  cfdh_exchange_fn cb_ex = nullptr;
  void *cb_user = nullptr;

  bool prof_on = false;
  ProfSlot prof[12];
  std::vector<hipEvent_t> ev_pool;
  struct EvRec { int kind; hipEvent_t a, b; };
  std::vector<EvRec> ev_pending;
  size_t ev_next = 0;

  cfdh_stats last_stats;
  long long n_allreduce = 0, n_halo = 0, n_host_sync = 0, n_krylov = 0, n_allgather = 0;
  long long n_attainable_stops = 0;
  long long n_pc_builds = 0;

  bool pcd_set = false, pcd_ready = false;
  int pcd_in = -1, pcd_out = -1, pcd_time = 0;
  double pcd_ct = 0;
  dbuf<int> pcd_iptr, pcd_inc, pcd_fptr, pcd_fac;
  dbuf<unsigned> pcd_islot, pcd_fslot;
  dbuf<int> pcd_sptr, pcd_scol, pcd_rlen;
  dbuf<double> pcd_K, pcd_mdinv, pcd_t, pcd_q;
  dbuf<float> pcd_Kf;
  dbuf<unsigned char> pcd_flag;
  std::vector<double> h_pcd_md;
  int ew_version = 0;
  double ew_rtol0 = 0.3, ew_rtol_max = 0.9, ew_gamma = 1.0, ew_alpha = 1.6180339887498949, ew_threshold = 0.1;
  std::vector<double> hist_fnorm, hist_rtol, hist_relres;
  std::vector<int> hist_its;
  double ksp_last_relres = 0;
  bool lean = true;
  struct SolveEnv {
    int krylov_fp32 = 1;
    bool guess_check = false;
    bool no_attainable_stop = false;
    int gs_refine_from = -1;
    int ksp_lag = KRING - 3;
    double gs_eta2 = 1e-6;
    int l_cycles = 1, a_cycles = 1;
    bool dl0_coarse_sweeps = false;
  } env;
  dbuf<double> qu;
  long long n_guess_projections = 0;
  int guess_last_rank = -1, guess_last_k = 0;
  long long n_iter_sync = 0;
  long long n_cycles = 0;
};

#define CFDH_MAX_PBND 8

inline bool cfdh_pre_takes_sell(const CsrDev &A, bool rule) { return rule && A.has_sell_weighted(); }
inline bool cfdh_post_takes_sell(const CsrDev &A, bool rule) { return rule && A.has_sell(); }
inline bool cfdh_prolong_takes_sell(const CsrDev &P, bool rule) { return rule && P.has_sell(); }
inline bool cfdh_dl0_rule_A(const cfdh_ctx *c) { return cfdh_sweep_sell(c->dl0.A.nnz, c->nvo); }
inline bool cfdh_dl0_rule_P(const cfdh_ctx *c) { return cfdh_sweep_sell(c->dl0.P.nnz, c->nv); }
inline bool cfdh_dl0_coarse_fused(const cfdh_ctx *c) { return c->hLg.fused && c->opt.amg_smooth_degree == 1 && !c->env.dl0_coarse_sweeps; }

int cfdh_fail(cfdh_ctx *c, int code, const char *fmt, ...);
#define HIPCHK(c, call)                                                                           \
  do {                                                                                            \
    hipError_t e_ = (call);                                                                       \
    if (e_ != hipSuccess) return cfdh_fail((c), CFDH_E_HIP, "%s: %s (%s:%d)", #call, hipGetErrorString(e_), \
                                           __FILE__, __LINE__);                                   \
  } while (0)
#define CHK(call)            \
  do {                       \
    int r_ = (call);         \
    if (r_ != 0) return r_;  \
  } while (0)

int cfdh_build_mesh(cfdh_ctx *c, int64_t nv, int64_t nvo, int64_t nc, const int32_t *cells, const double *coords,
                    int64_t nfac, const int32_t *fcell, const int32_t *flocal, const int32_t *fmarker);
bool cfdh_renumber_enabled();
int cfdh_alloc_reduction(cfdh_ctx *c, bool with_event);
int cfdh_upload_graph(cfdh_ctx *c);
int cfdh_upload_facets(cfdh_ctx *c);
int cfdh_alloc_dirichlet(cfdh_ctx *c);
int cfdh_alloc_state(cfdh_ctx *c);
int cfdh_alloc_precond_work(cfdh_ctx *c, size_t n, bool with_dinvA);
int cfdh_amg_setup(cfdh_ctx *c, AmgHier &H, const CsrHost &A, bool singular, int ncol);
int cfdh_level_setup(cfdh_ctx *c, AmgLevel &L, const CsrHost &A, double ratio, int ncol, std::vector<double> *w_out = nullptr);
int cfdh_upload_csr(cfdh_ctx *c, const CsrHost &H, CsrDev &D, const std::vector<double> *colw = nullptr, int parts = CFDH_UP_CSR | CFDH_UP_SELL);
int cfdh_aggregate_host_csr(const CsrHost &A, double theta, std::vector<int> &agg);

bool cfdh_amg_dev_enabled(const cfdh_ctx *c);
int cfdh_amg_setup_dev(cfdh_ctx *c, AmgHier &H, CsrDev &A0, bool singular, int ncol);
int cfdh_level_setup_dev(cfdh_ctx *c, AmgLevel &L, CsrDev &A, double ratio, int ncol);
int cfdh_proxy_dev(cfdh_ctx *c, CsrDev &out);
int cfdh_proxy_ras_dev(cfdh_ctx *c, CsrDev &out);
int cfdh_cc_h_dev(cfdh_ctx *c, double alpha, double beta, CsrDev &out);

#define CFDH3_MAX_SLOTS 320
int cfdh_build_mesh3(cfdh_ctx *c, int64_t nv, int64_t nvo, int64_t nc, const int32_t *cells, const double *coords,
                     int64_t nfac, const int32_t *fcell, const int32_t *flocal, const int32_t *fmarker);
int k3_upload_quadrature(cfdh_ctx *c);
int k3_moments(cfdh_ctx *c);
int k3_assemble(cfdh_ctx *c, const double *xstate, int mode);
int k3_spmv_full(cfdh_ctx *c, const double *x, double *y);
int k3_spmv_full_multi(cfdh_ctx *c, const double *X, double *Y, int ld, int nvec);
int k3_spmv_block(cfdh_ctx *c, int blk, const double *x, double *y, const double *b);
int k3_spmv_block_ghost(cfdh_ctx *c, int blk, const double *xv, double *y, const double *b);
int k3_nullspace_partials(cfdh_ctx *c, int nb);
int k3_functional_partials(cfdh_ctx *c, int kind, int marker, int nb);
int k3_wss(cfdh_ctx *c, double *out);

int kg_upload_tables(cfdh_ctx *c);
int cfdh_build_mesh_gen(cfdh_ctx *c, int etype, int64_t nv, int64_t nv_owned, int64_t nc, const int32_t *cells, const double *coords, int64_t nfac,
                        const int32_t *fcell, const int32_t *flocal, const int32_t *fmarker);
int cfdh_gen_element_stiffness(const cfdh_ctx *c, const int32_t *v, const double *X, double *K);
int cfdh_facet_nodes(const cfdh_ctx *c, int f, int out[3]);
int kg_assemble(cfdh_ctx *c, const double *xstate, int mode);
int kg_functional_partials(cfdh_ctx *c, int kind, int marker, int nb);
int kg_wss(cfdh_ctx *c, double *out);

int kg3_upload_tables(cfdh_ctx *c);
int cfdh_build_mesh_gen3(cfdh_ctx *c, int etype, int64_t nv, int64_t nv_owned, int64_t nc, const int32_t *cells, const double *coords, int64_t nfac,
                         const int32_t *fcell, const int32_t *flocal, const int32_t *fmarker);
int cfdh_gen3_element_stiffness(const cfdh_ctx *c, const int32_t *v, const double *X, double *K);
int cfdh_facet_nodes3(const cfdh_ctx *c, int f, int out[8]);
int kg3_assemble(cfdh_ctx *c, const double *xstate, int mode);
int kg3_functional_partials(cfdh_ctx *c, int kind, int marker, int nb);
int kg3_wss(cfdh_ctx *c, double *out);

int cfdh_pcd_supported(cfdh_ctx *c, const char *who);
int cfdh_pcd_setup(cfdh_ctx *c);
int k_pcd_assemble(cfdh_ctx *c, const double *xstate);
int k_pcd_apply(cfdh_ctx *c, const double *r, double *s);

int k_ipcs_wss(cfdh_ctx *c, double *out);
int k_ws_accumulate(cfdh_ctx *c, int n, double w, const double *tau);
int k_ws_derive(cfdh_ctx *c, int n, int which, double *out);

void prof_begin(cfdh_ctx *c, int kind);
void prof_end(cfdh_ctx *c, int kind);
void prof_flush(cfdh_ctx *c);
int k_upload_quadrature(cfdh_ctx *c);
int k_halo_pack(cfdh_ctx *c, const double *vec);
int k_moments(cfdh_ctx *c);
int k_assemble(cfdh_ctx *c, const double *xstate, int mode);
int k_spmv_full(cfdh_ctx *c, const double *x, double *y);
int k_spmv_full_multi(cfdh_ctx *c, const double *X, double *Y, int ld, int nvec);
int k_spmv_block(cfdh_ctx *c, int blk, const double *x, double *y, const double *b, double alpha);
int k_spmv_block_ghost(cfdh_ctx *c, int blk, const double *xv, double *y, const double *b);
int k_extract_diag(cfdh_ctx *c);
int k_cheb_a00(cfdh_ctx *c, const double *b, double *x);
int k_cheb_a00_coeffs(cfdh_ctx *c);
int k_cheb_init(cfdh_ctx *c, int n, const double *dinv, const double *b, double *d0, double *x, double itheta, int accumulate,
                const double *coef);
int k_nullspace_test(cfdh_ctx *c, double *nrm, double *absnrm);
int k_spmv_a01_keep(cfdh_ctx *c, const double *x, double *y, const double *b, double *q);
int k_spmv_full_kept(cfdh_ctx *c, const double *x, double *y, const double *q);
int k_resid_norm(cfdh_ctx *c, const double *x, const double *b, double *r, double *nrm, bool *done);
int k_fnorm_nulltest(cfdh_ctx *c, int n, const double *F, double *fn, double *nrm, double *absnrm);
int k_bc_scatter(cfdh_ctx *c, int n, int ncomp, const int *idx, const unsigned char *flag, const double *val, const double *mult);
int v_pack_state(cfdh_ctx *c, const double *u_user, const double *p_user, double *dst);
int k_functional(cfdh_ctx *c, int kind, int marker, double *out);
int k_wss(cfdh_ctx *c, double *out);

int k_csr_spmv(cfdh_ctx *c, const CsrDev &A, const double *x, double *y, int mode, const double *b);
int k_csr_spmv_ncol(cfdh_ctx *c, const CsrDev &A, const double *x, double *y, int mode, const double *b, int ncol);
int k_amg_vcycle(cfdh_ctx *c, AmgHier &H, const double *b, double *x);
int k_level_smooth(cfdh_ctx *c, AmgLevel *L, const double *b, double *x, int degree);
bool k_cc_cheb2_scale(cfdh_ctx *c, AmgLevel *L, const double *b, double *x, const double *ml, double *y);
int k_cc_scale(cfdh_ctx *c, int n, const double *ml, const double *z, double *y);
int k_dl0_down(cfdh_ctx *c, const double *halo_vec);
int k_dl0_up(cfdh_ctx *c, double *out);
int k_ext_pack(cfdh_ctx *c, const double *vec, double *out);
int k_scatter_global(cfdh_ctx *c, int n, const int *l2g, const double *loc, double *glob);
int k_gather_global(cfdh_ctx *c, int n, const int *l2g, const double *glob, double *loc);
int k_cc_combine(cfdh_ctx *c, int n, double alpha, double beta, const double *t, const double *z, const double *r, const unsigned char *pbc, double *out, double *out2 = nullptr);

int v_pointwise_mult(cfdh_ctx *c, int n, const double *a, const double *b, double *out);
int v_guess_combine(cfdh_ctx *c, int n, const double *U, const double *W, int ld, int k, const double *hd, const double *b, double *x, double *r);
// ... 56 lines not shown
```

### cfd_hemodynamic_amd/csrc/cfdh_setup.cpp

```cpp
#include <algorithm>
#include <chrono>
#include <cmath>
#include <cstdarg>
#include <cstdlib>
#include <numeric>

#include "cfdh_internal.hpp"
#include "cfdh_mesh_host.hpp"

int cfdh_fail(cfdh_ctx *c, int code, const char *fmt, ...) {
  char buf[512];
  va_list ap;
  va_start(ap, fmt);
  vsnprintf(buf, sizeof buf, fmt, ap);
  va_end(ap);
  extern std::string g_cfdh_last_error;
  g_cfdh_last_error = buf;
  if (c) c->err = buf;
  return code;
}

int cfdh_host_threads() {
  const char *e = getenv("CFDH_HOST_THREADS");
  int n = e ? atoi(e) : 8;
// ... 316 lines not shown
      int j = A.col[k];
      if (j != i && std::fabs(A.val[k]) >= theta * std::sqrt(d[i] * d[j])) scol.push_back(j);
    }
    sptr[i + 1] = (int)scol.size();
  }
  agg.assign(n, -1);
  int na = 0;
  for (int i = 0; i < n; i++) {
    if (agg[i] >= 0) continue;
    bool freeNb = sptr[i + 1] > sptr[i];
    for (int k = sptr[i]; k < sptr[i + 1] && freeNb; k++) if (agg[scol[k]] >= 0) freeNb = false;
    if (!freeNb) continue;
    agg[i] = na;
    for (int k = sptr[i]; k < sptr[i + 1]; k++) agg[scol[k]] = na;
    na++;
  }
  std::vector<int> agg2 = agg;
  for (int i = 0; i < n; i++) {
    if (agg[i] >= 0) continue;
    for (int k = sptr[i]; k < sptr[i + 1]; k++) if (agg[scol[k]] >= 0) { agg2[i] = agg[scol[k]]; break; }
  }
  agg.swap(agg2);
  for (int i = 0; i < n; i++) {
    if (agg[i] >= 0) continue;
    if (sptr[i + 1] == sptr[i]) continue;
    agg[i] = na;
    for (int k = sptr[i]; k < sptr[i + 1]; k++) if (agg[scol[k]] < 0) agg[scol[k]] = na;
    na++;
  }
  return na;
}

int cfdh_aggregate_host_csr(const CsrHost &A, double theta, std::vector<int> &agg) { return aggregate_host(A, theta, agg); }

static void spgemm_host(const CsrHost &A, const CsrHost &B, CsrHost &C) {
  C.n = A.n; C.m = B.m;
  C.rowptr.assign(A.n + 1, 0);
  std::vector<std::vector<int>> cols(A.n);
  std::vector<std::vector<double>> vals(A.n);
#pragma omp parallel num_threads(cfdh_host_threads())
  {
    std::vector<int> mark(B.m, -1), list;
    std::vector<double> acc(B.m, 0.0);
#pragma omp for schedule(dynamic, 256)
    for (int i = 0; i < A.n; i++) {
      list.clear();
      for (int k = A.rowptr[i]; k < A.rowptr[i + 1]; k++) {
        int j = A.col[k];
        double a = A.val[k];
        for (int k2 = B.rowptr[j]; k2 < B.rowptr[j + 1]; k2++) {
          int cc = B.col[k2];
          if (mark[cc] != i) { mark[cc] = i; acc[cc] = 0.0; list.push_back(cc); }
          acc[cc] += a * B.val[k2];
        }
      }
      std::sort(list.begin(), list.end());
      cols[i] = list;
      vals[i].resize(list.size());
      for (size_t t = 0; t < list.size(); t++) vals[i][t] = acc[list[t]];
    }
  }
  for (int i = 0; i < A.n; i++) C.rowptr[i + 1] = C.rowptr[i] + (int)cols[i].size();
  C.col.resize(C.rowptr[A.n]); C.val.resize(C.rowptr[A.n]);
  for (int i = 0; i < A.n; i++) {
    std::copy(cols[i].begin(), cols[i].end(), C.col.begin() + C.rowptr[i]);
    std::copy(vals[i].begin(), vals[i].end(), C.val.begin() + C.rowptr[i]);
  }
}

static void transpose_host(const CsrHost &A, CsrHost &T) {
  T.n = A.m; T.m = A.n;
  T.rowptr.assign(A.m + 1, 0);
  for (int k = 0; k < A.nnz(); k++) T.rowptr[A.col[k] + 1]++;
  for (int i = 0; i < A.m; i++) T.rowptr[i + 1] += T.rowptr[i];
  T.col.resize(A.nnz()); T.val.resize(A.nnz());
  std::vector<int> fill(T.rowptr.begin(), T.rowptr.end() - 1);
  for (int i = 0; i < A.n; i++)
    for (int k = A.rowptr[i]; k < A.rowptr[i + 1]; k++) { int p = fill[A.col[k]]++; T.col[p] = i; T.val[p] = A.val[k]; }
}

static int upload_csr(cfdh_ctx *c, const CsrHost &H, CsrDev &D, const std::vector<double> *colw = nullptr,
                      int parts = CFDH_UP_CSR | CFDH_UP_SELL) {
  D.n = H.n; D.m = H.m; D.nnz = H.nnz();
  if (parts & (CFDH_UP_CSR | CFDH_UP_CSRF)) {
    HIPCHK(c, D.rowptr.upload(H.rowptr, c->stream));
    HIPCHK(c, D.col.upload(H.col, c->stream));
  }
  if (parts & CFDH_UP_CSR) HIPCHK(c, D.val.upload(H.val, c->stream));
  if (parts & CFDH_UP_CSRF) {
    std::vector<float> vf(H.val.begin(), H.val.end());
    HIPCHK(c, D.valf.upload(vf, c->stream));
    HIPCHK(c, hipStreamSynchronize(c->stream));
  }
  if (!(parts & CFDH_UP_SELL)) { HIPCHK(c, hipStreamSynchronize(c->stream)); return 0; }
  const int ns = (H.n + 63) / 64;
  std::vector<int> sptr(ns + 1, 0);
  D.sell_maxw = 0;
#pragma omp parallel for schedule(static) num_threads(cfdh_host_threads()) if (ns > 256)
  for (int sl = 0; sl < ns; sl++) {
    int w = 0;
    for (int r = sl * 64; r < std::min(H.n, sl * 64 + 64); r++) w = std::max(w, H.rowptr[r + 1] - H.rowptr[r]);
    sptr[sl + 1] = 64 * w;
  }
  for (int sl = 0; sl < ns; sl++) { D.sell_maxw = std::max(D.sell_maxw, sptr[sl + 1] / 64); sptr[sl + 1] += sptr[sl]; }
  std::vector<int> scol((size_t)sptr[ns], 0);
  std::vector<float> sval((size_t)sptr[ns], 0.0f), svalw;
  if (colw) svalw.assign((size_t)sptr[ns], 0.0f);
#pragma omp parallel for schedule(static) num_threads(cfdh_host_threads()) if (H.n > 4096)
  for (int r = 0; r < H.n; r++) {
    const int sl = r >> 6, lane = r & 63;
    for (int k = H.rowptr[r], j = 0; k < H.rowptr[r + 1]; k++, j++) {
      const size_t p = (size_t)sptr[sl] + (size_t)j * 64 + lane;
      scol[p] = H.col[k]; sval[p] = (float)H.val[k];
      if (colw) svalw[p] = (float)(H.val[k] * (*colw)[H.col[k]]);
    }
  }
  D.nslice = ns;
  HIPCHK(c, D.sptr.upload(sptr, c->stream));
  HIPCHK(c, D.scol.upload(scol, c->stream));
  HIPCHK(c, D.sval.upload(sval, c->stream));
  if (colw) HIPCHK(c, D.svalw.upload(svalw, c->stream));
  HIPCHK(c, hipStreamSynchronize(c->stream));
  return 0;
}

static bool dense_inverse(std::vector<double> &a, int n) {
  std::vector<double> inv((size_t)n * n, 0.0);
  for (int i = 0; i < n; i++) inv[(size_t)i * n + i] = 1.0;
  for (int col = 0; col < n; col++) {
    int piv = col;
    double best = std::fabs(a[(size_t)col * n + col]);
    for (int r = col + 1; r < n; r++) if (std::fabs(a[(size_t)r * n + col]) > best) { best = std::fabs(a[(size_t)r * n + col]); piv = r; }
    if (!(best > 0)) return false;
    if (piv != col)
      for (int k = 0; k < n; k++) { std::swap(a[(size_t)piv * n + k], a[(size_t)col * n + k]); std::swap(inv[(size_t)piv * n + k], inv[(size_t)col * n + k]); }
    double d = 1.0 / a[(size_t)col * n + col];
    for (int k = 0; k < n; k++) { a[(size_t)col * n + k] *= d; inv[(size_t)col * n + k] *= d; }
#pragma omp parallel for schedule(static) num_threads(cfdh_host_threads()) if (n > 256)
    for (int r = 0; r < n; r++) {
      if (r == col) continue;
      double f = a[(size_t)r * n + col];
      if (f == 0.0) continue;
      for (int k = 0; k < n; k++) { a[(size_t)r * n + k] -= f * a[(size_t)col * n + k]; inv[(size_t)r * n + k] -= f * inv[(size_t)col * n + k]; }
    }
  }
  a.swap(inv);
  return true;
}

int cfdh_upload_csr(cfdh_ctx *c, const CsrHost &H, CsrDev &D, const std::vector<double> *colw, int parts) { return upload_csr(c, H, D, colw, parts); }

static void csr_axpby_scaled(const CsrHost &A, double alpha, const double *s_row, const double *s_col, const CsrHost &B, CsrHost &C) {
  C.n = A.n; C.m = A.m;
  C.rowptr.assign(A.n + 1, 0);
  const int nt = cfdh_host_threads();
#pragma omp parallel for schedule(static) num_threads(nt) if (A.n > 4096)
  for (int i = 0; i < A.n; i++) {
    int ka = A.rowptr[i], kb = B.rowptr[i], cnt = 0;
    const int ea = A.rowptr[i + 1], eb = B.rowptr[i + 1];
    while (ka < ea || kb < eb) {
      const int ja = ka < ea ? A.col[ka] : 0x7fffffff, jb = kb < eb ? B.col[kb] : 0x7fffffff;
      const int j = ja < jb ? ja : jb;
      if (ja == j) ka++;
      if (jb == j) kb++;
      cnt++;
    }
    C.rowptr[i + 1] = cnt;
  }
  for (int i = 0; i < A.n; i++) C.rowptr[i + 1] += C.rowptr[i];
  C.col.resize(C.rowptr[A.n]); C.val.resize(C.rowptr[A.n]);
// ... 227 lines not shown
```

### cfd_hemodynamic_amd/csrc/cfdh_solver.cpp

```cpp
#include <algorithm>
#include <chrono>
#include <cmath>

#include "cfdh_internal.hpp"
#include "cfdh_krylov_host.hpp"

int cfdh_host_threads();

static double wall_ms() {
  using namespace std::chrono;
  return duration<double, std::milli>(steady_clock::now().time_since_epoch()).count();
}

int cfdh_download_blocks(cfdh_ctx *c, std::vector<double> &a00, std::vector<double> &a01, std::vector<double> &a10,
                         std::vector<double> &a11) {
  const size_t nz = (size_t)c->nnzv, d = (size_t)c->dim;
  a00.resize(d * d * nz); a01.resize(d * nz); a10.resize(d * nz); a11.resize(nz);
  HIPCHK(c, hipMemcpyAsync(a00.data(), c->A00.p, sizeof(double) * d * d * nz, hipMemcpyDeviceToHost, c->stream));
  HIPCHK(c, hipMemcpyAsync(a01.data(), c->A01.p, sizeof(double) * d * nz, hipMemcpyDeviceToHost, c->stream));
  HIPCHK(c, hipMemcpyAsync(a10.data(), c->A10.p, sizeof(double) * d * nz, hipMemcpyDeviceToHost, c->stream));
  HIPCHK(c, hipMemcpyAsync(a11.data(), c->A11.p, sizeof(double) * nz, hipMemcpyDeviceToHost, c->stream));
  HIPCHK(c, hipStreamSynchronize(c->stream));
  return 0;
}
// ... 343 lines not shown
  const unsigned pbit = 1u << c->dim;
  for (int i = 0; i < nvo; i++) pbc[i] = (c->h_bcflag[i] & pbit) ? 1 : 0;
  const bool pcd = c->opt.pc_type == 2;
  if (pcd) mark_pcd_outlet(c, pbc);
  else if (!c->ds_terms || c->form == CFDH_FORM_ROTATIONAL) mark_outflow_nodes(c, pbc);
  if (pcd) CHK(upload_pcd_flags(c, pbc));
  if (!c->hL.valid || c->hL_pbc != pbc || c->hL_singular != c->singular) {
    CsrHost Lh;
    Lh.n = Lh.m = nvo;
    Lh.rowptr.assign(nvo + 1, 0);
    Lh.col.reserve(c->nnzv); Lh.val.reserve(c->nnzv);
    bool any_pbc = false;
    for (int i = 0; i < nvo; i++) {
      any_pbc |= pbc[i] != 0;
      if (pbc[i]) { Lh.col.push_back(i); Lh.val.push_back(1.0); }
      else
        for (int k = vp[i]; k < vp[i + 1]; k++) {
          const int w = vc[k];
          if (w >= nvo || pbc[w]) continue;
          Lh.col.push_back(w); Lh.val.push_back(c->h_Lval[k]);
        }
      Lh.rowptr[i + 1] = (int)Lh.col.size();
    }
    if (multi) CHK(amg_setup_from_host(c, c->hL, Lh, c->singular != 0 || !any_pbc, 1));
    else {
      CsrDev Ld;
      CHK(upload_csr_plain(c, Lh, Ld));
      CHK(cfdh_amg_setup_dev(c, c->hL, Ld, c->singular != 0 || !any_pbc, 1));
    }
    c->hL_pbc = pbc;
    c->hL_singular = c->singular;
    std::vector<double> ml(nvo);
    for (int i = 0; i < nvo; i++) ml[i] = pbc[i] ? 0.0 : c->h_Ml[i];
    HIPCHK(c, c->ccMl.upload(ml, c->stream));
    HIPCHK(c, c->ccPbc.upload(pbc, c->stream));
    HIPCHK(c, hipStreamSynchronize(c->stream));
  }
  if (multi) CHK(build_global_pressure(c));
  const double t2 = wall_ms();
  if (pcd) {
    HIPCHK(c, hipStreamSynchronize(c->stream));
    c->ms_pc_build_dev = wall_ms() - t0;
    return 0;
  }
  c->cc_alpha = c->rho * c->ts_a[0] / (c->ts_theta * c->dt);
  c->cc_beta = c->mu;
  {
    CsrDev Hd;
    CHK(cfdh_cc_h_dev(c, c->cc_alpha, c->cc_beta, Hd));
    CHK(cfdh_level_setup_dev(c, c->Hlev, Hd, 8.0, 1));
  }
  HIPCHK(c, hipStreamSynchronize(c->stream));
  c->ms_pc_build_dev = wall_ms() - t0;
  if (c->opt.verbose)
    fprintf(stderr, "[cfdh] preconditioner built on the device: velocity hierarchy %.1f ms, pressure Laplacian %.1f ms, H %.1f ms\n", t1 - t0, t2 - t1,
            wall_ms() - t2);
  return 0;
}
static int build_cc(cfdh_ctx *c) {
  static const bool host_multi = (getenv("CFDH_AMG_HOST_MULTI") && getenv("CFDH_AMG_HOST_MULTI")[0] == '1') ||
                                 (getenv("CFDH_PC_HOST_ASSEMBLY") && getenv("CFDH_PC_HOST_ASSEMBLY")[0] == '1');
  if (c->nranks > 1 && cfdh_amg_dev_enabled(c) && !host_multi) return build_cc_dev(c);
  if (c->nranks == 1 && cfdh_amg_dev_enabled(c)) {
    const int rc = build_cc_dev(c);
    if (rc == 0) return 0;
    if (c->opt.verbose) fprintf(stderr, "[cfdh] device-side hierarchy set-up failed (%s): host build\n", c->err.c_str());
    c->hL.clear(); c->hA.clear();
  }
  return build_cc_host(c);
}

int cfdh_pc_update(cfdh_ctx *c, bool refresh_amg) {
  const int nu = c->dim * c->nvo;
  if (c->opt.pc_type == 2) {
    CHK(cfdh_pcd_supported(c, "pc_type 2"));
    if (!c->pcd_set) return cfdh_fail(c, CFDH_E_STATE, "pc_type 2 (PCD) needs cfdh_set_schur_pcd");
  } else if (c->dim == 3 && c->opt.pc_type != 1) {
    return cfdh_fail(c, CFDH_E_ARG, "tetrahedral contexts support pc_type 1 and 2 only");
  }
  if (c->opt.pc_type == 1 || c->opt.pc_type == 2) {
    if (refresh_amg || !c->pc_valid) {
      c->pc_graph_valid = false;
      CHK(build_cc(c));
      c->pc_valid = true;
      c->pc_its_ref = 0;
      c->steps_since_refresh = 0;
      c->last_stats.pc_refreshes++;
    c->n_pc_builds++;
    }
    if (c->opt.pc_type == 2) CHK(k_pcd_assemble(c, c->x.p));
    return 0;
  }
  CHK(k_extract_diag(c));
  double *v = c->pu0.p, *w = c->pu1.p;
  CHK(v_copy(c, nu, c->prand.p, v));
  double lam = 1.0;
  for (int it = 0; it < 8; it++) {
    CHK(k_spmv_block(c, 1, v, w, nullptr, 0));
    CHK(v_pointwise_mult(c, nu, w, c->dinvA.p, w));
    CHK(v_norm_to_dev(c, nu, w, c->red_out.p + RO_POWER));
    CHK(v_scale_inv_dev(c, nu, w, c->red_out.p + RO_POWER, v));
  }
  CHK(scalars_read(c, ScalarRead{c->red_out.p + RO_POWER, 1, false}, &lam, false));
  if (!(lam > 0) || !std::isfinite(lam)) return cfdh_fail(c, CFDH_E_DIVERGED, "non-finite spectral estimate of D^-1 A00 (NaN in the Jacobian?)");
  c->lmaxA = 1.15 * lam;
  CHK(k_cheb_a00_coeffs(c));
  if (refresh_amg || !c->pc_valid) {
    c->pc_graph_valid = false;
    CsrHost S;
    CHK(build_schur_host(c, S));
    bool any_pbc = false;
    for (int i = 0; i < c->nvo; i++) any_pbc |= (c->h_bcflag[i] & (1u << c->dim)) != 0;
    CHK(cfdh_amg_setup(c, c->hS, S, c->singular != 0 || !any_pbc, 1));
    c->pc_valid = true;
    c->pc_its_ref = 0;
    c->steps_since_refresh = 0;
    c->last_stats.pc_refreshes++;
    c->n_pc_builds++;
  }
  return 0;
}

static bool ras_ghost_rhs() {
  static const bool on = !(getenv("CFDH_RAS_GHOST_RHS") && getenv("CFDH_RAS_GHOST_RHS")[0] == '0');
  return on;
}

static bool lean_newton(const cfdh_ctx *c) {
  return c->lean && c->nranks == 1 && c->nv == c->nvo && c->dim == 2 && !c->gen;
}
static bool lean_scope(const cfdh_ctx *c) { return lean_newton(c) && (c->opt.pc_type == 1 || c->opt.pc_type == 2); }
static bool lean_keep_qu(const cfdh_ctx *c) { return lean_scope(c) && c->opt.schur_full != 0 && !c->singular && c->qu.p != nullptr; }

static int pressure_cycle_combine(cfdh_ctx *c, double alpha, double beta, const double *zH, const double *r, const unsigned char *flag,
                                  double *out, double *out2) {
  const int nvo = c->nvo;
  if (c->env.l_cycles > 1 && c->hL.lev.size() >= 1 && c->hL.lev[0]->A.val.p) {
    AmgLevel *L0 = c->hL.lev[0];
    CHK(k_amg_vcycle(c, c->hL, c->pu1.p, c->pu2.p));
    for (int cyc = 1; cyc < c->env.l_cycles; cyc++) {
      CHK(k_csr_spmv(c, L0->A, c->pu2.p, L0->r.p, 1, c->pu1.p));
      CHK(k_amg_vcycle(c, c->hL, L0->r.p, L0->d0.p));
      CHK(v_axpy(c, nvo, 1.0, L0->d0.p, c->pu2.p));
    }
    CHK(k_cc_combine(c, nvo, alpha, beta, c->pu2.p, zH, r, flag, out));
    return out2 ? v_copy(c, nvo, out, out2) : 0;
  }
  c->epi.on = true; c->epi.done = false;
  c->epi.alpha = alpha; c->epi.beta = beta; c->epi.zH = zH; c->epi.r = r;
  c->epi.pbc = flag; c->epi.out = out;
  const int rc = k_amg_vcycle(c, c->hL, c->pu1.p, c->pu2.p);
  c->epi.on = false;
  CHK(rc);
  if (!c->epi.done) return k_cc_combine(c, nvo, alpha, beta, c->pu2.p, zH, r, flag, out, out2);
  c->epi.done = false;
  return out2 ? v_copy(c, nvo, out, out2) : 0;
}

static int pcd_stage(cfdh_ctx *c, const double *r, double *z, int stage) {
  const int nvo = c->nvo, nu = c->dim * nvo;
  const double *ru = r, *rp = r + nu;
  double *zu = z, *zp = z + nu;
  const bool upper = c->opt.schur_full == 2;
  switch (stage) {
    case 0:
      if (!upper) CHK(k_amg_vcycle(c, c->hA, ru, c->pu0.p));
      return 0;
    case 1:
      if (!upper) CHK(k_spmv_block(c, 3, c->pu0.p, c->pp0.p, rp, 0));
      return k_pcd_apply(c, upper ? rp : c->pp0.p, c->pu1.p);
    case 2:
      return pressure_cycle_combine(c, 1.0, c->mu, c->pcd_t.p, c->pcd_q.p, c->pcd_flag.p, zp, nullptr);
    case 3:
      if (c->opt.schur_full) {
        if (lean_keep_qu(c)) CHK(k_spmv_a01_keep(c, zp, c->pu0.p, ru, c->qu.p));
        else CHK(k_spmv_block(c, 2, zp, c->pu0.p, ru, 0));
        CHK(k_amg_vcycle(c, c->hA, c->pu0.p, zu));
      } else {
        CHK(v_copy(c, nu, c->pu0.p, zu));
      }
      return 0;
    default:
      return 0;
  }
}

static int pc_stage(cfdh_ctx *c, const double *r, double *z, int stage) {
  const int nvo = c->nvo, nu = c->dim * nvo;
  const double *ru = r, *rp = r + nu;
  double *zu = z, *zp = z + nu;
  const bool multi = c->nranks > 1;
  const bool global_p = c->gp_n > 0 && multi;
  if (c->opt.pc_type == 2) return pcd_stage(c, r, z, stage);
  if (c->opt.pc_type == 1) {
    const bool upper = c->opt.schur_full == 2;
    const bool dist = global_p && c->dl0.on;
// ... 789 lines not shown
```

### include/cfdh.h

```cpp
#ifndef CFDH_H
#define CFDH_H

#include <stdint.h>

#ifdef __cplusplus
extern "C" {
#endif

#define CFDH_ABI_VERSION 1

enum {
  CFDH_OK = 0,
  CFDH_E_ARG = -1,
  CFDH_E_HIP = -2,
  CFDH_E_STATE = -3,
  CFDH_E_DIVERGED = -4,
  CFDH_E_COMM = -5,
  CFDH_E_NOMEM = -6
};

enum {
  CFDH_CONVERGED_FNORM_ABS = 2,
  CFDH_CONVERGED_FNORM_RELATIVE = 3,
  CFDH_CONVERGED_SNORM_RELATIVE = 4,
// ... 21 lines not shown
  int32_t schur_full;
  int32_t amg_smooth_degree;
  double amg_smooth_ratio;
  double amg_theta;
  int32_t amg_max_coarse;
  int32_t pc_refresh;
  int32_t remove_p_mean;
  int32_t verbose;
  int32_t pc_type;
  int32_t cc_smooth_degree;
  int32_t ksp_guess;
} cfdh_options;

typedef struct cfdh_stats {
  int32_t newton_its, krylov_its, reason, pc_refreshes;
  double fnorm0, fnorm;
  double ms_assemble, ms_solve, ms_pc_setup, ms_total;
} cfdh_stats;


int cfdh_create(cfdh_ctx **out, int device, int gdim, int64_t nv, int64_t nv_owned, int64_t nc,
                const int32_t *cells, const double *coords, int64_t nfacets, const int32_t *facet_cells,
                const int32_t *facet_local, const int32_t *facet_marker);
enum { CFDH_ELEM_P1 = 0, CFDH_ELEM_P2_TRIANGLE = 1, CFDH_ELEM_Q1_QUADRILATERAL = 2, CFDH_ELEM_P1_GENERIC = 3 };
int cfdh_create_elem(cfdh_ctx **out, int device, int gdim, int elem, int64_t nn, int64_t nc, const int32_t *cells,
                     const double *node_coords, int64_t nfacets, const int32_t *facet_cells, const int32_t *facet_local,
                     const int32_t *facet_marker);
int cfdh_create_elem_part(cfdh_ctx **out, int device, int gdim, int elem, int64_t nn, int64_t nn_owned, int64_t nc, const int32_t *cells,
                          const double *node_coords, int64_t nfacets, const int32_t *facet_cells, const int32_t *facet_local,
                          const int32_t *facet_marker);
int cfdh_set_facet_markers(cfdh_ctx *ctx, int64_t nfacets, const int32_t *markers);
void cfdh_destroy(cfdh_ctx *ctx);
const char *cfdh_last_error(const cfdh_ctx *ctx);
int cfdh_abi_version(void);

int cfdh_set_params(cfdh_ctx *ctx, double dt, double rho, double mu, double mu_facet, const double f[3]);
int cfdh_default_options(cfdh_options *opt);
int cfdh_set_options(cfdh_ctx *ctx, const cfdh_options *opt);


int cfdh_clear_dirichlet(cfdh_ctx *ctx);
int cfdh_add_dirichlet(cfdh_ctx *ctx, int field, int64_t n, const int32_t *nodes, const double *values);
int cfdh_update_dirichlet(cfdh_ctx *ctx, int field, int64_t n, const int32_t *nodes, const double *values);


int cfdh_set_state(cfdh_ctx *ctx, const double *u_prev, const double *p_prev, const double *u, const double *p);
int cfdh_get_solution(cfdh_ctx *ctx, double *u, double *p);
int cfdh_get_previous(cfdh_ctx *ctx, double *u_prev, double *p_prev);
int cfdh_get_residual(cfdh_ctx *ctx, double *ru, double *rp);
int cfdh_advance(cfdh_ctx *ctx);
int cfdh_advance_field(cfdh_ctx *ctx, int field);


int cfdh_set_time_scheme(cfdh_ctx *ctx, double theta, double a0, double a1, double a2);

int cfdh_set_boundary_terms(cfdh_ctx *ctx, int ds_terms, int backflow_marker, double beta);


enum { CFDH_FORM_CONVECTIVE = 0, CFDH_FORM_ROTATIONAL = 1 };
int cfdh_set_formulation(cfdh_ctx *ctx, int form);
int cfdh_set_pressure_boundaries(cfdh_ctx *ctx, int n, const int32_t *markers, const double *values, double beta_nitsche);
int cfdh_set_pressure_boundaries_ex(cfdh_ctx *ctx, int n, const int32_t *markers, const double *values, double beta_nitsche,
                                    const uint8_t *nitsche, const double *beta_backflow);


int cfdh_set_schur_pcd(cfdh_ctx *ctx, int inlet_marker, int outlet_marker, int time_term);
int cfdh_set_ksp_forcing(cfdh_ctx *ctx, int version, double rtol_0, double rtol_max, double gamma, double alpha, double threshold);
int cfdh_get_newton_history(cfdh_ctx *ctx, int32_t *n, double *fnorm, double *ksp_rtol, int32_t *ksp_its, double *ksp_rel_res);
int cfdh_get_pcd_operator(cfdh_ctx *ctx, int64_t *nnz, int32_t *rowptr, int32_t *col, double *vals, double *mass_diag);
int cfdh_apply_preconditioner(cfdh_ctx *ctx, const double *r, double *z);
int cfdh_apply_operator(cfdh_ctx *ctx, const double *r, double *z, double *w);

#define CFDH_AMG_HIER_A 0
#define CFDH_AMG_HIER_P 1
#define CFDH_AMG_HIER_H 2
#define CFDH_AMG_HIER_PG 3
#define CFDH_AMG_HIER_DL0 4
#define CFDH_AMG_OP_A 0
#define CFDH_AMG_OP_P 1
#define CFDH_AMG_OP_G 2
#define CFDH_AMG_OP_SB 3
#define CFDH_AMG_OP_SC 4
#define CFDH_AMG_OP_PT 5
int cfdh_get_amg_operator(cfdh_ctx *ctx, int hier, int level, int which, int64_t *nrow, int64_t *ncol, int64_t *nnz, int32_t *rowptr,
                          int32_t *col, double *vals);
#define CFDH_AMG_VEC_DINV 0
#define CFDH_AMG_VEC_WDINV 1
#define CFDH_AMG_VEC_AGG 2
#define CFDH_AMG_VEC_COARSE_INV 3
#define CFDH_AMG_VEC_D 4
#define CFDH_AMG_VEC_LAMBDA 5
#define CFDH_AMG_VEC_CC_SCALARS 6
#define CFDH_AMG_VEC_CC_ML 7
#define CFDH_AMG_VEC_CC_PBC 8
#define CFDH_AMG_VEC_SPGEMM_ROWS 9
#define CFDH_AMG_VEC_SHAPE 10
#define CFDH_AMG_VEC_ORDER 11
#define CFDH_AMG_VEC_A00_LMAX 12
#define CFDH_AMG_VEC_A00_DINV 13
#define CFDH_AMG_VEC_DL0_SHAPE 14
int cfdh_get_amg_vectors(cfdh_ctx *ctx, int hier, int level, int which, int64_t *n, double *out);

#define CFDH_KVOP_DOT 0
#define CFDH_KVOP_NORM2 1
#define CFDH_KVOP_NORM2_PAIR 2
#define CFDH_KVOP_NORM2_TRIPLE 3
#define CFDH_KVOP_NORMINF_DIFF 4
#define CFDH_KVOP_SUB_MEAN 5
#define CFDH_KVOP_NORM_SCALE_INV 6
#define CFDH_KVOP_MULTIDOT 7
#define CFDH_KVOP_MULTIDOT32 8
#define CFDH_KVOP_GRAM 9
#define CFDH_KVOP_MULTIAXPY 10
#define CFDH_KVOP_LINCOMB 11
#define CFDH_KVOP_LINCOMB_KEEP 12
#define CFDH_KVOP_GS_UPDATE_NORMALIZE 13
#define CFDH_KVOP_GS_UPDATE32 14
#define CFDH_KVOP_STORE32 15
#define CFDH_KVOP_GUESS 16
#define CFDH_KVOP_AXPY 17
#define CFDH_KVOP_WAXPY 18
#define CFDH_KVOP_SCALE 19
#define CFDH_KVOP_SCALE_TO 20
#define CFDH_KVOP_PMULT 21
#define CFDH_KVOP_COUNT 22
int cfdh_krylov_vec_op(cfdh_ctx *ctx, int op, int n, int ld, int nvec, const double *A, const double *B, const double *x, const double *y,
                       const double *coef, double scalar, int flags, double *out1, double *out2, float *out32, int32_t *nscal,
                       double *scal_host, double *scal_dev, double *scal_mirror);


int cfdh_create_ipcs(cfdh_ctx **out, int device, int gdim, int64_t nn, int64_t nvert, int64_t nc, const int32_t *cells,
                     const double *node_coords, int64_t nfacets, const int32_t *facet_cells, const int32_t *facet_local,
                     const int32_t *facet_marker);
int cfdh_ipcs_set_form(cfdh_ctx *ctx, double conv_coeff, double force_coeff);
int cfdh_ipcs_set_tolerances(cfdh_ctx *ctx, const double rtol[3], double atol, const int32_t max_it[3]);
typedef struct cfdh_ipcs_stats {
  int32_t its[3], reason[3];
  double rel_res[3];
  double ms_assemble, ms_solve[3], ms_total;
  int32_t launches, host_syncs;
} cfdh_ipcs_stats;
int cfdh_ipcs_step(cfdh_ctx *ctx, cfdh_ipcs_stats *stats);
int cfdh_ipcs_get_operator(cfdh_ctx *ctx, int which, int64_t *nnz, int32_t *rowptr, int32_t *col, double *vals);
int cfdh_ipcs_get_intermediate(cfdh_ctx *ctx, int which, double *out);
int cfdh_ipcs_apply_pressure_pc(cfdh_ctx *ctx, const double *r, double *z);
#define CFDH_IPCS_NSCAL 16
int cfdh_ipcs_krylov_solve(cfdh_ctx *ctx, int which, const double *b, const double *x0, double rtol, double atol, int max_it,
                           double *x, cfdh_ipcs_stats *stats, double *scalars);

int cfdh_set_previous2(cfdh_ctx *ctx, const double *u_prev2);
int cfdh_get_previous2(cfdh_ctx *ctx, double *u_prev2);
int cfdh_shift_history(cfdh_ctx *ctx);


int cfdh_assemble(cfdh_ctx *ctx, int want_jacobian);
int cfdh_get_csr(cfdh_ctx *ctx, int64_t *nnz, int32_t *rowptr, int32_t *col, double *vals);
int cfdh_spmv(cfdh_ctx *ctx, const double *x, double *y);


int cfdh_solve_step(cfdh_ctx *ctx, cfdh_stats *stats);

int cfdh_functional(cfdh_ctx *ctx, int kind, int marker, double *out);

int cfdh_wall_shear_stress(cfdh_ctx *ctx, double *shear);

int cfdh_wall_stats_reset(cfdh_ctx *ctx);
// ... 26 lines not shown
```

Baseline: 441.8.

## Compress AMG fine-level column indices to 16-bit offsets from per-slice base

Result: faster. 446.6 (median of 6 runs) (+1.1%).

```diff
diff --git a/cfd_hemodynamic_amd/_lib.py b/cfd_hemodynamic_amd/_lib.py
--- a/cfd_hemodynamic_amd/_lib.py
+++ b/cfd_hemodynamic_amd/_lib.py
@@ -179,6 +179,7 @@
 AMG_HIER_A, AMG_HIER_P, AMG_HIER_H = 0, 1, 2
 AMG_HIER_PG, AMG_HIER_DL0 = 3, 4
 AMG_OP_A, AMG_OP_P, AMG_OP_G, AMG_OP_SB, AMG_OP_SC, AMG_OP_PT = 0, 1, 2, 3, 4, 5
+AMG_OP_COL16 = 0x100
 (AMG_VEC_DINV, AMG_VEC_WDINV, AMG_VEC_AGG, AMG_VEC_COARSE_INV, AMG_VEC_D, AMG_VEC_LAMBDA, AMG_VEC_CC_SCALARS, AMG_VEC_CC_ML,
  AMG_VEC_CC_PBC, AMG_VEC_SPGEMM_ROWS, AMG_VEC_SHAPE, AMG_VEC_ORDER, AMG_VEC_A00_LMAX, AMG_VEC_A00_DINV, AMG_VEC_DL0_SHAPE) = range(15)
 IP_RHO, IP_RHO_OLD, IP_ALPHA, IP_OMEGA, IP_BETA, IP_RZ, IP_TOL2, IP_BN2, IP_RN2, IP_DONE, IP_ITS, IP_BAD = range(12)
diff --git a/cfd_hemodynamic_amd/csrc/cfdh_amg_apply.hip b/cfd_hemodynamic_amd/csrc/cfdh_amg_apply.hip
--- a/cfd_hemodynamic_amd/csrc/cfdh_amg_apply.hip
+++ b/cfd_hemodynamic_amd/csrc/cfdh_amg_apply.hip
@@ -26,13 +26,37 @@
 __device__ __forceinline__ double wsum(double v) { return wave_sum(v); }
 __device__ __forceinline__ double2 wsum(double2 v) { return make_double2(wave_sum(v.x), wave_sum(v.y)); }
 
-template <int MAXW, typename T>
+template <int MAXW, typename T, bool C16 = false>
 __device__ __forceinline__ T sell_row_dot(const int *__restrict__ sp, const int *__restrict__ sc, const float *__restrict__ sv,
-                                          const T *__restrict__ x, int sl, int lane, T a) {
+                                          const T *__restrict__ x, int sl, int lane, T a, const int *__restrict__ sb = nullptr,
+                                          const unsigned short *__restrict__ sh = nullptr) {
   sl = __builtin_amdgcn_readfirstlane(sl);
   const int p0 = sp[sl], w = (sp[sl + 1] - p0) >> 6;
   int cidx[MAXW];
   float cval[MAXW];
+  if constexpr (C16) {
+    const int base = sb[sl];
+    const bool narrow = base >= 0;
+    const int add = narrow ? base : 0;
+    if (narrow) {
+#pragma unroll
+      for (int k = 0; k < MAXW; k++)
+        if (k < w) { const int p = p0 + k * 64 + lane; cidx[k] = (int)NTLOAD(sh + p); cval[k] = NTLOAD(sv + p); }
+    } else {
+#pragma unroll
+      for (int k = 0; k < MAXW; k++)
+        if (k < w) { const int p = p0 + k * 64 + lane; cidx[k] = NTLOAD(sc + p); cval[k] = NTLOAD(sv + p); }
+    }
+    T g[MAXW];
+#pragma unroll
+    for (int k = 0; k < MAXW; k++)
+      if (k < w) g[k] = x[cidx[k] + add];
+#pragma unroll
+    for (int k = 0; k < MAXW; k++)
+      if (k < w) a = vfma((double)cval[k], g[k], a);
+    for (int k = MAXW; k < w; k++) { const int p = p0 + k * 64 + lane; a = vfma((double)sv[p], x[narrow ? base + (int)sh[p] : sc[p]], a); }
+    return a;
+  }
 #pragma unroll
   for (int k = 0; k < MAXW; k++)
     if (k < w) { const int p = p0 + k * 64 + lane; cidx[k] = NTLOAD(sc + p); cval[k] = NTLOAD(sv + p); }
@@ -175,17 +199,19 @@
 }
 int k_level_smooth(cfdh_ctx *c, AmgLevel *L, const double *b, double *x, int degree) { return level_cheb(c, L, b, x, true, degree, false); }
 
+template <bool C16>
 __global__ __launch_bounds__(TPB) void sell_cheb2_scale_kernel(int n, const int *__restrict__ sptr, const int *__restrict__ scol,
                                                                const float *__restrict__ svalw, const double *__restrict__ wdinv,
                                                                const double *__restrict__ dinv, const double *__restrict__ b,
                                                                double *__restrict__ x, const double *__restrict__ ml,
-                                                               double *__restrict__ y, double c1, double c2) {
+                                                               double *__restrict__ y, double c1, double c2,
+                                                               const int *__restrict__ sbase, const unsigned short *__restrict__ scol16) {
   const int row = blockIdx.x * TPB + threadIdx.x;
   if (row >= n) return;
   const int sl = row >> 6, lane = row & 63;
   const int p0 = sptr[sl], w = (sptr[sl + 1] - p0) >> 6;
   (void)p0; (void)w;
-  const double a = sell_row_dot<10, double>(sptr, scol, svalw, b, sl, lane, 0.0);
+  const double a = sell_row_dot<10, double, C16>(sptr, scol, svalw, b, sl, lane, 0.0, sbase, scol16);
   const double bi = b[row];
   const double dd = wdinv[row] * bi;
   const double xv = dd + (c1 * dd + c2 * dinv[row] * (bi - a));
@@ -198,8 +224,12 @@
   const double theta = 0.5 * (L->lmax + L->lmin), delta = 0.5 * (L->lmax - L->lmin), sigma = theta / delta;
   const double rho = 1.0 / sigma, rho_new = 1.0 / (2.0 * sigma - rho);
   const double c1 = rho_new * rho, c2 = 2.0 * rho_new / delta;
-  hipLaunchKernelGGL(sell_cheb2_scale_kernel, dim3((n + TPB - 1) / TPB), dim3(TPB), 0, c->stream, n, L->A.sptr.p, L->A.scol.p,
-                     L->A.svalw.p, L->wdinv.p, L->dinv.p, b, x, ml, y, c1, c2);
+  if (L->A.has_sell16())
+    hipLaunchKernelGGL(sell_cheb2_scale_kernel<true>, dim3((n + TPB - 1) / TPB), dim3(TPB), 0, c->stream, n, L->A.sptr.p, L->A.scol.p,
+                       L->A.svalw.p, L->wdinv.p, L->dinv.p, b, x, ml, y, c1, c2, L->A.sbase.p, L->A.scol16.p);
+  else
+    hipLaunchKernelGGL(sell_cheb2_scale_kernel<false>, dim3((n + TPB - 1) / TPB), dim3(TPB), 0, c->stream, n, L->A.sptr.p, L->A.scol.p,
+                       L->A.svalw.p, L->wdinv.p, L->dinv.p, b, x, ml, y, c1, c2, (const int *)nullptr, (const unsigned short *)nullptr);
   return hipGetLastError() == hipSuccess;
 }
 
@@ -386,9 +416,10 @@
 __device__ __forceinline__ d3 epi_apply(d3 acc, int, double, double, const double *, const double *, const unsigned char *) { return acc; }
 __device__ __forceinline__ d3 epi_value(d3 acc, unsigned, double, double, double, double) { return acc; }
 
-template <int LPR, typename VT, typename T>
+template <int LPR, typename VT, typename T, bool C16>
 __global__ __launch_bounds__(TPB) void fused_down_kernel(int n, const int *__restrict__ rowptr, const int *__restrict__ col,
-                                                         const VT *__restrict__ val, const T *__restrict__ x, T *__restrict__ y) {
+                                                         const VT *__restrict__ val, const T *__restrict__ x, T *__restrict__ y,
+                                                         const int *__restrict__ rbase, const unsigned short *__restrict__ col16) {
   const int gid = blockIdx.x * TPB + threadIdx.x;
   const int row = gid / LPR, l = gid % LPR;
   T a = vzero((const T *)nullptr);
@@ -396,6 +427,24 @@
     const int ks = rowptr[row], ke = rowptr[row + 1];
     int cidx[4];
     VT cval[4];
+    if constexpr (C16) {
+      const int base = rbase[row];
+      const bool narrow = base >= 0;
+      const int add = narrow ? base : 0;
+      if (narrow) {
+#pragma unroll
+        for (int q = 0; q < 4; q++) { const int k = ks + l + q * LPR; if (k < ke) { cidx[q] = (int)col16[k]; cval[q] = val[k]; } }
+      } else {
+#pragma unroll
+        for (int q = 0; q < 4; q++) { const int k = ks + l + q * LPR; if (k < ke) { cidx[q] = col[k]; cval[q] = val[k]; } }
+      }
+      T g[4];
+#pragma unroll
+      for (int q = 0; q < 4; q++) { const int k = ks + l + q * LPR; if (k < ke) g[q] = x[cidx[q] + add]; }
+#pragma unroll
+      for (int q = 0; q < 4; q++) { const int k = ks + l + q * LPR; if (k < ke) a = vfma((double)cval[q], g[q], a); }
+      for (int k = ks + l + 4 * LPR; k < ke; k += LPR) a = vfma((double)val[k], x[narrow ? base + (int)col16[k] : col[k]], a);
+    } else {
 #pragma unroll
     for (int q = 0; q < 4; q++) { const int k = ks + l + q * LPR; if (k < ke) { cidx[q] = col[k]; cval[q] = val[k]; } }
     T g[4];
@@ -404,6 +453,7 @@
 #pragma unroll
     for (int q = 0; q < 4; q++) { const int k = ks + l + q * LPR; if (k < ke) a = vfma((double)cval[q], g[q], a); }
     for (int k = ks + l + 4 * LPR; k < ke; k += LPR) a = vfma((double)val[k], x[col[k]], a);
+    }
   }
   a = lsum<LPR>(a);
   if (row < n && l == 0) y[row] = a;
@@ -446,13 +496,15 @@
   a = g8(a);
   if (row < n && l == 0) x[row] = epbc ? epi_apply(a, row, ea, eb, ezH, er, epbc) : a;
 }
-template <typename T, bool WIDE>
+struct Col16Sell { const int *baseB; const unsigned short *hB; const int *baseC; const unsigned short *hC; };
+template <typename T, bool WIDE, bool C16>
 __global__ __launch_bounds__(TPB) void fused_up_sell_kernel(int n, const int *__restrict__ spB, const int *__restrict__ scB,
                                                             const float *__restrict__ svB, const T *__restrict__ b,
                                                             const int *__restrict__ spC, const int *__restrict__ scC,
                                                             const float *__restrict__ svC, const T *__restrict__ xc,
                                                             T *__restrict__ x, double ea, double eb, const double *__restrict__ ezH,
-                                                            const double *__restrict__ er, const unsigned char *__restrict__ epbc) {
+                                                            const double *__restrict__ er, const unsigned char *__restrict__ epbc,
+                                                            Col16Sell c16) {
   const int row = blockIdx.x * TPB + threadIdx.x;
   if (row >= n) return;
   const int sl = __builtin_amdgcn_readfirstlane(row >> 6), lane = row & 63;
@@ -465,26 +517,40 @@
   int pC = 0, wC = 0;
   if (spC) { pC = spC[sl]; wC = (spC[sl + 1] - pC) >> 6; }
   const int wmax = wB > wC ? wB : wC;
+  int baseB = -1, baseC = -1;
+  if constexpr (C16) { baseB = c16.baseB[sl]; if (spC) baseC = c16.baseC[sl]; }
+  const bool nB = baseB >= 0, nC = baseC >= 0;
+  const int addB = nB ? baseB : 0, addC = nC ? baseC : 0;
   for (int k0 = 0; k0 < (WIDE ? wmax : 1); k0 += MW) {
     int cB[MW], cC[MW];
     float vB[MW], vC[MW];
+    if (C16 && nB) {
+#pragma unroll
+      for (int k = 0; k < MW; k++) if (k0 + k < wB) { const int p = pB + (k0 + k) * 64 + lane; cB[k] = (int)NTLOAD(c16.hB + p); vB[k] = NTLOAD(svB + p); }
+    } else {
 #pragma unroll
     for (int k = 0; k < MW; k++) if (k0 + k < wB) { const int p = pB + (k0 + k) * 64 + lane; cB[k] = NTLOAD(scB + p); vB[k] = NTLOAD(svB + p); }
+    }
+    if (C16 && nC) {
+#pragma unroll
+      for (int k = 0; k < MW; k++) if (k0 + k < wC) { const int p = pC + (k0 + k) * 64 + lane; cC[k] = (int)NTLOAD(c16.hC + p); vC[k] = NTLOAD(svC + p); }
+    } else {
 #pragma unroll
     for (int k = 0; k < MW; k++) if (k0 + k < wC) { const int p = pC + (k0 + k) * 64 + lane; cC[k] = NTLOAD(scC + p); vC[k] = NTLOAD(svC + p); }
+    }
     T gB[MW], gC[MW];
 #pragma unroll
-    for (int k = 0; k < MW; k++) if (k0 + k < wB) gB[k] = b[cB[k]];
-#pragma unroll
-    for (int k = 0; k < MW; k++) if (k0 + k < wC) gC[k] = xc[cC[k]];
+    for (int k = 0; k < MW; k++) if (k0 + k < wB) gB[k] = b[C16 ? cB[k] + addB : cB[k]];
+#pragma unroll
+    for (int k = 0; k < MW; k++) if (k0 + k < wC) gC[k] = xc[C16 ? cC[k] + addC : cC[k]];
 #pragma unroll
     for (int k = 0; k < MW; k++) if (k0 + k < wB) a = vfma((double)vB[k], gB[k], a);
 #pragma unroll
     for (int k = 0; k < MW; k++) if (k0 + k < wC) a = vfma((double)vC[k], gC[k], a);
   }
   if (!WIDE) {
-    for (int k = MW; k < wB; k++) { const int p = pB + k * 64 + lane; a = vfma((double)svB[p], b[scB[p]], a); }
-    for (int k = MW; k < wC; k++) { const int p = pC + k * 64 + lane; a = vfma((double)svC[p], xc[scC[p]], a); }
+    for (int k = MW; k < wB; k++) { const int p = pB + k * 64 + lane; a = vfma((double)svB[p], b[(C16 && nB) ? baseB + (int)c16.hB[p] : scB[p]], a); }
+    for (int k = MW; k < wC; k++) { const int p = pC + k * 64 + lane; a = vfma((double)svC[p], xc[(C16 && nC) ? baseC + (int)c16.hC[p] : scC[p]], a); }
   }
   x[row] = epbc ? epi_value(a, e_f, ea, eb, e_zh, e_r) : a;
 }
@@ -511,15 +577,17 @@
   if (row < n && l == 0) x[row] = a;
 }
 
-template <typename VT, typename T>
+template <typename VT, typename T, bool C16 = false>
 static void launch_down(cfdh_ctx *c, const CsrDev &G, const VT *val, const T *x, T *y) {
   const long long avg = G.n > 0 ? (G.nnz + G.n - 1) / G.n : 1;
   const int lpr = avg > 96 ? 64 : (avg > 48 ? 32 : (avg > 20 ? 16 : 8));
   dim3 block(TPB), grid((unsigned)(((long long)G.n * lpr + TPB - 1) / TPB));
-  if (lpr == 64) hipLaunchKernelGGL((fused_down_kernel<64, VT, T>), grid, block, 0, c->stream, G.n, G.rowptr.p, G.col.p, val, x, y);
-  else if (lpr == 32) hipLaunchKernelGGL((fused_down_kernel<32, VT, T>), grid, block, 0, c->stream, G.n, G.rowptr.p, G.col.p, val, x, y);
-  else if (lpr == 16) hipLaunchKernelGGL((fused_down_kernel<16, VT, T>), grid, block, 0, c->stream, G.n, G.rowptr.p, G.col.p, val, x, y);
-  else hipLaunchKernelGGL((fused_down_kernel<8, VT, T>), grid, block, 0, c->stream, G.n, G.rowptr.p, G.col.p, val, x, y);
+  const int *rb = C16 ? G.rbase.p : nullptr;
+  const unsigned short *c16 = C16 ? G.col16.p : nullptr;
+  if (lpr == 64) hipLaunchKernelGGL((fused_down_kernel<64, VT, T, C16>), grid, block, 0, c->stream, G.n, G.rowptr.p, G.col.p, val, x, y, rb, c16);
+  else if (lpr == 32) hipLaunchKernelGGL((fused_down_kernel<32, VT, T, C16>), grid, block, 0, c->stream, G.n, G.rowptr.p, G.col.p, val, x, y, rb, c16);
+  else if (lpr == 16) hipLaunchKernelGGL((fused_down_kernel<16, VT, T, C16>), grid, block, 0, c->stream, G.n, G.rowptr.p, G.col.p, val, x, y, rb, c16);
+  else hipLaunchKernelGGL((fused_down_kernel<8, VT, T, C16>), grid, block, 0, c->stream, G.n, G.rowptr.p, G.col.p, val, x, y, rb, c16);
 }
 
 template <typename T>
@@ -529,7 +597,10 @@
     AmgLevel *L = H.lev[l], *N = H.lev[l + 1];
     const T *src = l == l0 ? b : (const T *)L->b.p;
     if (prof && l == 0) prof_begin(c, prof + 4);
-    if (L->fine) launch_down<float, T>(c, L->G, L->G.valf.p, src, (T *)N->b.p);
+    constexpr bool one_rhs = sizeof(T) == sizeof(double);
+    if (one_rhs && L->fine && l == 0 && L->G.has_csr16()) {
+      if constexpr (one_rhs) launch_down<float, T, true>(c, L->G, L->G.valf.p, src, (T *)N->b.p);
+    } else if (L->fine) launch_down<float, T>(c, L->G, L->G.valf.p, src, (T *)N->b.p);
     else launch_down<double, T>(c, L->G, L->G.val.p, src, (T *)N->b.p);
     if (prof && l == 0) prof_end(c, prof + 4);
   }
@@ -550,10 +621,10 @@
       if (H.coarse_n > 0)
         hipLaunchKernelGGL((dense_mv_kernel<T>), dim3(H.coarse_n), dim3(64), 0, c->stream, H.coarse_n, H.coarse_inv.p, bl, xl);
       else if (L->sell)
-        hipLaunchKernelGGL((fused_up_sell_kernel<T, true>), dim3((unsigned)((L->n + TPB - 1) / TPB)), dim3(TPB), 0, c->stream, L->n,
+        hipLaunchKernelGGL((fused_up_sell_kernel<T, true, false>), dim3((unsigned)((L->n + TPB - 1) / TPB)), dim3(TPB), 0, c->stream, L->n,
                            L->Sb.sptr.p, L->Sb.scol.p, L->Sb.sval.p, bl, (const int *)nullptr, (const int *)nullptr,
                            (const float *)nullptr, (const T *)nullptr, xl, 0.0, 0.0, (const double *)nullptr, (const double *)nullptr,
-                           (const unsigned char *)nullptr);
+                           (const unsigned char *)nullptr, Col16Sell{nullptr, nullptr, nullptr, nullptr});
       else
         hipLaunchKernelGGL((fused_up_csr_kernel<T>), dim3((unsigned)((8ll * L->n + TPB - 1) / TPB)), dim3(TPB), 0, c->stream, L->n,
                            L->Sb.rowptr.p, L->Sb.col.p, L->Sb.val.p, bl, (const int *)nullptr, (const int *)nullptr,
@@ -573,18 +644,22 @@
     if (epi) { xl = (T *)c->epi.out; c->epi.done = true; }
     const int nrow = (l == 0 && c->up0_rows > 0 && c->up0_rows < L->n) ? c->up0_rows : L->n;
     if (prof && l == 0) prof_begin(c, prof);
-    if (L->sell && L->Sb.sell_maxw <= 14 && L->Sc.sell_maxw <= 14)
-      hipLaunchKernelGGL((fused_up_sell_kernel<T, false>), dim3((unsigned)((nrow + TPB - 1) / TPB)), dim3(TPB), 0, c->stream, nrow,
-                         L->Sb.sptr.p, L->Sb.scol.p, L->Sb.sval.p, bl, L->Sc.sptr.p, L->Sc.scol.p, L->Sc.sval.p, (const T *)N->x.p, xl,
-                         ea, eb, ezH, er, epbc);
-    else if (L->sell)
-      hipLaunchKernelGGL((fused_up_sell_kernel<T, true>), dim3((unsigned)((nrow + TPB - 1) / TPB)), dim3(TPB), 0, c->stream, nrow,
-                         L->Sb.sptr.p, L->Sb.scol.p, L->Sb.sval.p, bl, L->Sc.sptr.p, L->Sc.scol.p, L->Sc.sval.p, (const T *)N->x.p, xl,
-                         ea, eb, ezH, er, epbc);
-    else
+    constexpr bool one_rhs = sizeof(T) == sizeof(double);
+    const bool c16 = one_rhs && l == 0 && L->sell && L->Sb.has_sell16() && L->Sc.has_sell16();
+    const Col16Sell h16 = c16 ? Col16Sell{L->Sb.sbase.p, L->Sb.scol16.p, L->Sc.sbase.p, L->Sc.scol16.p} : Col16Sell{nullptr, nullptr, nullptr, nullptr};
+#define UP_SELL(WIDE, C16)                                                                                                                  \
+  hipLaunchKernelGGL((fused_up_sell_kernel<T, WIDE, C16>), dim3((unsigned)((nrow + TPB - 1) / TPB)), dim3(TPB), 0, c->stream, nrow,         \
+                     L->Sb.sptr.p, L->Sb.scol.p, L->Sb.sval.p, bl, L->Sc.sptr.p, L->Sc.scol.p, L->Sc.sval.p, (const T *)N->x.p, xl, ea, eb, \
+                     ezH, er, epbc, h16)
+    if (L->sell && L->Sb.sell_maxw <= 14 && L->Sc.sell_maxw <= 14) {
+      if (c16) { if constexpr (one_rhs) UP_SELL(false, true); } else UP_SELL(false, false);
+    } else if (L->sell) {
+      if (c16) { if constexpr (one_rhs) UP_SELL(true, true); } else UP_SELL(true, false);
+    } else
       hipLaunchKernelGGL((fused_up_csr_kernel<T>), dim3((unsigned)((8ll * nrow + TPB - 1) / TPB)), dim3(TPB), 0, c->stream, nrow,
                          L->Sb.rowptr.p, L->Sb.col.p, L->Sb.val.p, bl, L->Sc.rowptr.p, L->Sc.col.p, L->Sc.val.p, (const T *)N->x.p, xl,
                          ea, eb, ezH, er, epbc);
+#undef UP_SELL
     if (prof && l == 0) prof_end(c, prof);
   }
   HIPCHK(c, hipGetLastError());
diff --git a/cfd_hemodynamic_amd/csrc/cfdh_api.cpp b/cfd_hemodynamic_amd/csrc/cfdh_api.cpp
--- a/cfd_hemodynamic_amd/csrc/cfdh_api.cpp
+++ b/cfd_hemodynamic_amd/csrc/cfdh_api.cpp
@@ -4,6 +4,7 @@
 
 #include <dlfcn.h>
 
+#include "cfdh_col16.hpp"
 #include "cfdh_internal.hpp"
 #include "cfdh_ipcs.hpp"
 
@@ -101,6 +102,13 @@
   cfdh_default_options(&c->opt);
   { const char *e = getenv("CFDH_NO_GRAPH"); c->use_graph = !(e && e[0] == '1'); }
   { const char *e = getenv("CFDH_SOLVE_LEAN"); c->lean = !(e && e[0] == '0'); }
+  { const char *e = getenv("CFDH_COL16"); c->col16 = !(e && e[0] == '0'); }
+  if (const char *e = getenv("CFDH_COL16_SPAN")) {
+    int v[3] = {65535, 65535, 65535};
+    const int got = sscanf(e, "%d,%d,%d", &v[0], &v[1], &v[2]);
+    if (got == 1) v[1] = v[2] = v[0];
+    if (got == 1 || got == 3) for (int k = 0; k < 3; k++) c->col16_span[k] = std::min(std::max(v[k], 0), 65535);
+  }
   {
     cfdh_ctx::SolveEnv &v = c->env;
     const char *e;
@@ -853,6 +861,8 @@
   AmgLevel *L = nullptr;
   CHK(amg_pick(c, "cfdh_get_amg_operator", hier, level, &H, &L));
   const bool dl0 = hier == CFDH_AMG_HIER_DL0;
+  const bool want16 = (which & CFDH_AMG_OP_COL16) != 0;
+  which &= ~CFDH_AMG_OP_COL16;
   if (dl0 ? (which != CFDH_AMG_OP_A && which != CFDH_AMG_OP_P && which != CFDH_AMG_OP_PT) : (which < CFDH_AMG_OP_A || which > CFDH_AMG_OP_SC))
     return cfdh_fail(c, CFDH_E_ARG, "cfdh_get_amg_operator: unknown operator %d", which);
   if (!H || dl0) level = 0;
@@ -860,6 +870,8 @@
                         : which == CFDH_AMG_OP_A ? L->A : which == CFDH_AMG_OP_P ? L->P : which == CFDH_AMG_OP_G ? L->G : which == CFDH_AMG_OP_SB ? L->Sb : L->Sc;
   if (M.n <= 0 || !M.rowptr.p || !M.col.p || !M.val.p)
     return cfdh_fail(c, CFDH_E_STATE, "cfdh_get_amg_operator: operator %d of level %d is not kept in fp64 CSR (P: CFDH_AMG_KEEP=1 before the build)", which, level);
+  if (want16 && !M.has_sell16() && !M.has_csr16())
+    return cfdh_fail(c, CFDH_E_STATE, "cfdh_get_amg_operator: operator %d of level %d has no 16-bit column copy", which, level);
   *nrow = M.n; *ncol = M.m; *nnz = M.nnz;
   if (!rowptr && !col && !vals) return 0;
   if (!rowptr || !col || !vals) return cfdh_fail(c, CFDH_E_ARG, "pass all of rowptr/col/vals or none");
@@ -872,6 +884,28 @@
   }
   HIPCHK(c, hipStreamSynchronize(c->stream));
   if (rp[M.n] != M.nnz) return cfdh_fail(c, CFDH_E_STATE, "cfdh_get_amg_operator: rowptr ends at %d, the operator holds %d entries", rp[M.n], M.nnz);
+  if (want16) {
+    auto fetch = [&](const void *src, size_t bytes, void *dst) -> int {
+      if (bytes) HIPCHK(c, hipMemcpyAsync(dst, src, bytes, hipMemcpyDeviceToHost, c->stream));
+      return 0;
+    };
+    std::vector<int> dec(cl.size());
+    if (M.has_sell16()) {
+      std::vector<int> sp((size_t)M.nslice + 1), sc(M.scol.n), sb((size_t)M.nslice);
+      std::vector<uint16_t> s16(M.scol16.n);
+      CHK(fetch(M.sptr.p, sizeof(int) * sp.size(), sp.data())); CHK(fetch(M.scol.p, sizeof(int) * sc.size(), sc.data()));
+      CHK(fetch(M.sbase.p, sizeof(int) * sb.size(), sb.data())); CHK(fetch(M.scol16.p, sizeof(uint16_t) * s16.size(), s16.data()));
+      HIPCHK(c, hipStreamSynchronize(c->stream));
+      cfdh_col16::sell_decode(M.n, rp.data(), sp.data(), sc.data(), sb.data(), s16.data(), dec.data());
+    } else {
+      std::vector<int> rb((size_t)M.n);
+      std::vector<uint16_t> c16(M.col16.n);
+      CHK(fetch(M.rbase.p, sizeof(int) * rb.size(), rb.data())); CHK(fetch(M.col16.p, sizeof(uint16_t) * c16.size(), c16.data()));
+      HIPCHK(c, hipStreamSynchronize(c->stream));
+      cfdh_col16::csr_decode(M.n, rp.data(), cl.data(), rb.data(), c16.data(), dec.data());
+    }
+    cl.swap(dec);
+  }
   const bool local0 = level == 0 && hier != CFDH_AMG_HIER_PG;
   const bool rows0 = local0 && which != CFDH_AMG_OP_G && which != CFDH_AMG_OP_PT && amg_local_dim(c, M.n);
   const bool cols0 = local0 && (which == CFDH_AMG_OP_A || which == CFDH_AMG_OP_SB || which == CFDH_AMG_OP_G || which == CFDH_AMG_OP_PT) && amg_local_dim(c, M.m);
@@ -1509,6 +1543,17 @@
     case 23: { const AmgHier &h = c->opt.pc_type >= 1 ? c->hL : c->hS; return h.lev.size() > 1 ? h.lev[1]->n : 0; }
     case 24: return c->hA.lev.size() > 1 ? c->hA.lev[1]->n : 0;
     case 25: { const AmgHier &h = c->opt.pc_type >= 1 ? c->hL : c->hS; return h.fused ? 1 : 0; }
+    case 91: case 92: case 93: case 94: case 95: case 96: case 97: case 98: case 99: case 100: case 101: case 102: {
+      const int k = (what - 91) / 2, hi = k / 3, op = k % 3;
+      const AmgHier &h = hi == 0 ? c->hA : (c->opt.pc_type >= 1 ? c->hL : c->hS);
+      if (!h.valid || h.lev.empty()) return 0;
+      const AmgLevel *L = h.lev[0];
+      const CsrDev &M = op == 0 ? L->Sb : op == 1 ? L->Sc : L->G;
+      return M.c16_count[(what - 91) & 1];
+    }
+    case 103: case 104: return c->Hlev.A.c16_count[what - 103];
+    case 105: return c->col16 ? 1 : 0;
+    case 106: case 107: case 108: return c->col16_span[what - 106];
     default: return -1;
   }
 }
diff --git a/cfd_hemodynamic_amd/csrc/cfdh_col16.hip b/cfd_hemodynamic_amd/csrc/cfdh_col16.hip
--- /dev/null
+++ b/cfd_hemodynamic_amd/csrc/cfdh_col16.hip
@@ -0,0 +1,89 @@
+#include <hip/hip_runtime.h>
+
+#include "cfdh_col16.hpp"
+#include "cfdh_internal.hpp"
+#include "cfdh_wave.hpp"
+
+namespace {
+using namespace cfdh_col16;
+
+__global__ __launch_bounds__(64) void sell_col16_kernel(int n, const int *__restrict__ rowptr, const int *__restrict__ sptr,
+                                                        const int *__restrict__ scol, int span, int *__restrict__ sbase,
+                                                        unsigned short *__restrict__ scol16, int *__restrict__ count) {
+  const int sl = blockIdx.x, lane = threadIdx.x, r = sl * 64 + lane;
+  Range g = r < n ? sell_row_range(rowptr, sptr, scol, r) : range_empty();
+#pragma unroll
+  for (int d = 32; d > 0; d >>= 1) g = range_join(g, Range{__shfl_xor(g.lo, d), __shfl_xor(g.hi, d)});
+  const int base = base_of(g, span);
+  if (lane == 0) { sbase[sl] = base; atomicAdd(count + (base >= 0 ? 0 : 1), 1); }
+  sell_row_encode(n, rowptr, sptr, scol, sl, lane, base, scol16);
+}
+__global__ __launch_bounds__(TPB) void csr_col16_kernel(int n, const int *__restrict__ rowptr, const int *__restrict__ col, int span,
+                                                        int *__restrict__ rbase, unsigned short *__restrict__ col16, int *__restrict__ count) {
+  const int r = blockIdx.x * TPB + threadIdx.x;
+  int base = 0;
+  if (r < n) {
+    base = rbase[r] = base_of(csr_row_range(rowptr, col, r), span);
+    csr_row_encode(rowptr, col, r, base, col16);
+  }
+  const unsigned long long live = __ballot(r < n), narrow = __ballot(r < n && base >= 0);
+  if ((threadIdx.x & 63) == 0) {
+    if (narrow) atomicAdd(count, __popcll(narrow));
+    if (live & ~narrow) atomicAdd(count + 1, __popcll(live & ~narrow));
+  }
+}
+
+int sell_copy(cfdh_ctx *c, CsrDev &M, int span, int *cnt) {
+  M.drop_col16();
+  if (!M.has_sell() && !M.has_sell_weighted()) return 0;
+  if (!M.rowptr.p || M.n <= 0 || M.nslice != (M.n + 63) / 64) return 0;
+  HIPCHK(c, M.sbase.alloc((size_t)M.nslice));
+  HIPCHK(c, M.scol16.alloc(M.scol.n));
+  hipLaunchKernelGGL(sell_col16_kernel, dim3(M.nslice), dim3(64), 0, c->stream, M.n, M.rowptr.p, M.sptr.p, M.scol.p, span, M.sbase.p,
+                     M.scol16.p, cnt);
+  HIPCHK(c, hipGetLastError());
+  return 0;
+}
+int csr_copy(cfdh_ctx *c, CsrDev &M, int span, int *cnt) {
+  M.drop_col16();
+  if (!M.rowptr.p || !M.col.p || !M.valf.p || M.n <= 0) return 0;
+  HIPCHK(c, M.rbase.alloc((size_t)M.n));
+  HIPCHK(c, M.col16.alloc(M.col.n));
+  hipLaunchKernelGGL(csr_col16_kernel, dim3((M.n + TPB - 1) / TPB), dim3(TPB), 0, c->stream, M.n, M.rowptr.p, M.col.p, span, M.rbase.p,
+                     M.col16.p, cnt);
+  HIPCHK(c, hipGetLastError());
+  return 0;
+}
+}
+
+int cfdh_col16_build(cfdh_ctx *c) {
+  AmgHier *hs[2] = {&c->hA, c->opt.pc_type >= 1 ? &c->hL : &c->hS};
+  const bool on = c->col16 && c->nranks == 1;
+  dbuf<int> cnt;
+  HIPCHK(c, cnt.alloc(14));
+  HIPCHK(c, cnt.zero(c->stream));
+  CsrDev *ops[7] = {nullptr, nullptr, nullptr, nullptr, nullptr, nullptr, nullptr};
+  for (int h = 0; h < 2; h++) {
+    AmgHier &H = *hs[h];
+    if (!H.valid || H.lev.empty()) continue;
+    AmgLevel *L = H.lev[0];
+    ops[3 * h] = &L->Sb; ops[3 * h + 1] = &L->Sc; ops[3 * h + 2] = &L->G;
+    const bool cycle = on && H.fused && H.lev.size() >= 2 && H.ncol == 1;
+    if (cycle && L->sell) { CHK(sell_copy(c, L->Sb, c->col16_span[0], cnt.p + 6 * h)); CHK(sell_copy(c, L->Sc, c->col16_span[1], cnt.p + 6 * h + 2)); }
+    else { L->Sb.drop_col16(); L->Sc.drop_col16(); }
+    if (cycle && L->fine) CHK(csr_copy(c, L->G, c->col16_span[2], cnt.p + 6 * h + 4));
+    else L->G.drop_col16();
+  }
+  if (c->opt.pc_type == 1 && c->Hlev.n > 0) {
+    CsrDev &A = c->Hlev.A;
+    ops[6] = &A;
+    if (on && cfdh_cheb2_sell(A.nnz, c->Hlev.n) && A.has_sell_weighted()) CHK(sell_copy(c, A, c->col16_span[0], cnt.p + 12));
+    else A.drop_col16();
+  }
+  int h_cnt[14];
+  HIPCHK(c, hipMemcpyAsync(h_cnt, cnt.p, sizeof h_cnt, hipMemcpyDeviceToHost, c->stream));
+  HIPCHK(c, hipStreamSynchronize(c->stream));
+  for (int k = 0; k < 7; k++)
+    if (ops[k] && (ops[k]->has_sell16() || ops[k]->has_csr16())) { ops[k]->c16_count[0] = h_cnt[2 * k]; ops[k]->c16_count[1] = h_cnt[2 * k + 1]; }
+  return 0;
+}
diff --git a/cfd_hemodynamic_amd/csrc/cfdh_col16.hpp b/cfd_hemodynamic_amd/csrc/cfdh_col16.hpp
--- /dev/null
+++ b/cfd_hemodynamic_amd/csrc/cfdh_col16.hpp
@@ -0,0 +1,80 @@
+#pragma once
+#include <cstdint>
+
+#ifndef CFDH_HD
+#ifdef __HIPCC__
+#define CFDH_HD __host__ __device__
+#else
+#define CFDH_HD
+#endif
+#endif
+
+namespace cfdh_col16 {
+
+constexpr int SPAN_MAX = 65535;
+
+CFDH_HD inline int clamp_span(long long span) { return span < 0 ? 0 : (span > SPAN_MAX ? SPAN_MAX : (int)span); }
+
+struct Range { int lo, hi; };
+CFDH_HD inline Range range_empty() { return Range{2147483647, -1}; }
+CFDH_HD inline Range range_add(Range r, int col) { return Range{col < r.lo ? col : r.lo, col > r.hi ? col : r.hi}; }
+CFDH_HD inline Range range_join(Range a, Range b) { return Range{a.lo < b.lo ? a.lo : b.lo, a.hi > b.hi ? a.hi : b.hi}; }
+CFDH_HD inline int base_of(Range r, int span) {
+  if (r.lo > r.hi) return 0;
+  return (long long)r.hi - (long long)r.lo <= (long long)clamp_span(span) ? r.lo : -1;
+}
+CFDH_HD inline uint16_t encode(int col, int base) { return (uint16_t)(col - base); }
+CFDH_HD inline int decode(uint16_t off, int base) { return base + (int)off; }
+
+CFDH_HD inline Range sell_row_range(const int *rowptr, const int *sptr, const int *scol, int r) {
+  Range g = range_empty();
+  const long long p0 = (long long)sptr[r >> 6] + (r & 63);
+  for (int k = 0, len = rowptr[r + 1] - rowptr[r]; k < len; k++) g = range_add(g, scol[p0 + 64ll * k]);
+  return g;
+}
+CFDH_HD inline void sell_row_encode(int n, const int *rowptr, const int *sptr, const int *scol, int sl, int lane, int base, uint16_t *scol16) {
+  const int r = sl * 64 + lane;
+  const int w = (sptr[sl + 1] - sptr[sl]) >> 6, len = r < n ? rowptr[r + 1] - rowptr[r] : 0;
+  const long long p0 = (long long)sptr[sl] + lane;
+  for (int k = 0; k < w; k++) scol16[p0 + 64ll * k] = (base >= 0 && k < len) ? encode(scol[p0 + 64ll * k], base) : (uint16_t)0;
+}
+CFDH_HD inline Range csr_row_range(const int *rowptr, const int *col, int r) {
+  Range g = range_empty();
+  for (int k = rowptr[r]; k < rowptr[r + 1]; k++) g = range_add(g, col[k]);
+  return g;
+}
+CFDH_HD inline void csr_row_encode(const int *rowptr, const int *col, int r, int base, uint16_t *col16) {
+  for (int k = rowptr[r]; k < rowptr[r + 1]; k++) col16[k] = base >= 0 ? encode(col[k], base) : (uint16_t)0;
+}
+
+inline void sell_convert(int n, const int *rowptr, const int *sptr, const int *scol, int span, int *sbase, uint16_t *scol16, int count[2]) {
+  count[0] = count[1] = 0;
+  for (int sl = 0, ns = (n + 63) / 64; sl < ns; sl++) {
+    Range g = range_empty();
+    for (int r = sl * 64; r < n && r < sl * 64 + 64; r++) g = range_join(g, sell_row_range(rowptr, sptr, scol, r));
+    const int base = sbase[sl] = base_of(g, span);
+    count[base >= 0 ? 0 : 1]++;
+    for (int lane = 0; lane < 64; lane++) sell_row_encode(n, rowptr, sptr, scol, sl, lane, base, scol16);
+  }
+}
+inline void csr_convert(int n, const int *rowptr, const int *col, int span, int *rbase, uint16_t *col16, int count[2]) {
+  count[0] = count[1] = 0;
+  for (int r = 0; r < n; r++) {
+    const int base = rbase[r] = base_of(csr_row_range(rowptr, col, r), span);
+    count[base >= 0 ? 0 : 1]++;
+    csr_row_encode(rowptr, col, r, base, col16);
+  }
+}
+inline void sell_decode(int n, const int *rowptr, const int *sptr, const int *scol, const int *sbase, const uint16_t *scol16, int *out) {
+  for (int r = 0; r < n; r++) {
+    const int base = sbase[r >> 6];
+    const long long p0 = (long long)sptr[r >> 6] + (r & 63);
+    for (int k = rowptr[r], j = 0; k < rowptr[r + 1]; k++, j++) out[k] = base >= 0 ? decode(scol16[p0 + 64ll * j], base) : scol[p0 + 64ll * j];
+  }
+}
+inline void csr_decode(int n, const int *rowptr, const int *col, const int *rbase, const uint16_t *col16, int *out) {
+  for (int r = 0; r < n; r++)
+    for (int k = rowptr[r]; k < rowptr[r + 1]; k++) out[k] = rbase[r] >= 0 ? decode(col16[k], rbase[r]) : col[k];
+}
+
+}
diff --git a/cfd_hemodynamic_amd/csrc/cfdh_internal.hpp b/cfd_hemodynamic_amd/csrc/cfdh_internal.hpp
--- a/cfd_hemodynamic_amd/csrc/cfdh_internal.hpp
+++ b/cfd_hemodynamic_amd/csrc/cfdh_internal.hpp
@@ -85,10 +85,17 @@
   dbuf<float> valf;
   bool has_sell() const { return sptr.p && scol.p && sval.p; }
   bool has_sell_weighted() const { return sptr.p && scol.p && svalw.p; }
+  dbuf<int> sbase, rbase;
+  dbuf<unsigned short> scol16, col16;
+  int c16_count[2] = {0, 0};
+  bool has_sell16() const { return sbase.p && scol16.p; }
+  bool has_csr16() const { return rbase.p && col16.p; }
+  void drop_col16() { sbase.release(); rbase.release(); scol16.release(); col16.release(); c16_count[0] = c16_count[1] = 0; }
 };
 enum { CFDH_UP_CSR = 1, CFDH_UP_SELL = 2, CFDH_UP_CSRF = 4};
 
-inline bool cfdh_short_rows(long long nnz, int n, int per_row) { return nnz <= (long long)per_row * n && n >= 16384; }
+inline int cfdh_sell_min_rows() { const char *e = getenv("CFDH_SELL_MIN_ROWS"); return e && atoi(e) > 0 ? atoi(e) : 16384; }
+inline bool cfdh_short_rows(long long nnz, int n, int per_row) { return nnz <= (long long)per_row * n && n >= cfdh_sell_min_rows(); }
 inline bool cfdh_level_fine(int dim, long long nnz, int n) { return cfdh_short_rows(nnz, n, dim == 3 ? 20 : 12); }
 inline bool cfdh_level_sell(int dim, long long nnz, int n, int ncol) {
   return cfdh_level_fine(dim, nnz, n) && (cfdh_short_rows(nnz, n, 12) || ncol == 1);
@@ -368,6 +375,8 @@
   std::vector<int> hist_its;
   double ksp_last_relres = 0;
   bool lean = true;
+  bool col16 = true;
+  int col16_span[3] = {65535, 65535, 65535};
   struct SolveEnv {
     int krylov_fp32 = 1;
     bool guess_check = false;
@@ -427,6 +436,8 @@
 int cfdh_proxy_dev(cfdh_ctx *c, CsrDev &out);
 int cfdh_proxy_ras_dev(cfdh_ctx *c, CsrDev &out);
 int cfdh_cc_h_dev(cfdh_ctx *c, double alpha, double beta, CsrDev &out);
+
+int cfdh_col16_build(cfdh_ctx *c);
 
 #define CFDH3_MAX_SLOTS 320
 int cfdh_build_mesh3(cfdh_ctx *c, int64_t nv, int64_t nvo, int64_t nc, const int32_t *cells, const double *coords,
diff --git a/cfd_hemodynamic_amd/csrc/cfdh_setup.cpp b/cfd_hemodynamic_amd/csrc/cfdh_setup.cpp
--- a/cfd_hemodynamic_amd/csrc/cfdh_setup.cpp
+++ b/cfd_hemodynamic_amd/csrc/cfdh_setup.cpp
@@ -422,10 +422,8 @@
 static int upload_csr(cfdh_ctx *c, const CsrHost &H, CsrDev &D, const std::vector<double> *colw = nullptr,
                       int parts = CFDH_UP_CSR | CFDH_UP_SELL) {
   D.n = H.n; D.m = H.m; D.nnz = H.nnz();
-  if (parts & (CFDH_UP_CSR | CFDH_UP_CSRF)) {
-    HIPCHK(c, D.rowptr.upload(H.rowptr, c->stream));
-    HIPCHK(c, D.col.upload(H.col, c->stream));
-  }
+  HIPCHK(c, D.rowptr.upload(H.rowptr, c->stream));
+  if (parts & (CFDH_UP_CSR | CFDH_UP_CSRF)) HIPCHK(c, D.col.upload(H.col, c->stream));
   if (parts & CFDH_UP_CSR) HIPCHK(c, D.val.upload(H.val, c->stream));
   if (parts & CFDH_UP_CSRF) {
     std::vector<float> vf(H.val.begin(), H.val.end());
diff --git a/cfd_hemodynamic_amd/csrc/cfdh_solver.cpp b/cfd_hemodynamic_amd/csrc/cfdh_solver.cpp
--- a/cfd_hemodynamic_amd/csrc/cfdh_solver.cpp
+++ b/cfd_hemodynamic_amd/csrc/cfdh_solver.cpp
@@ -449,6 +449,7 @@
     if (refresh_amg || !c->pc_valid) {
       c->pc_graph_valid = false;
       CHK(build_cc(c));
+      CHK(cfdh_col16_build(c));
       c->pc_valid = true;
       c->pc_its_ref = 0;
       c->steps_since_refresh = 0;
@@ -479,6 +480,7 @@
     bool any_pbc = false;
     for (int i = 0; i < c->nvo; i++) any_pbc |= (c->h_bcflag[i] & (1u << c->dim)) != 0;
     CHK(cfdh_amg_setup(c, c->hS, S, c->singular != 0 || !any_pbc, 1));
+    CHK(cfdh_col16_build(c));
     c->pc_valid = true;
     c->pc_its_ref = 0;
     c->steps_since_refresh = 0;
diff --git a/include/cfdh.h b/include/cfdh.h
--- a/include/cfdh.h
+++ b/include/cfdh.h
@@ -127,6 +127,7 @@
 #define CFDH_AMG_OP_SB 3
 #define CFDH_AMG_OP_SC 4
 #define CFDH_AMG_OP_PT 5
+#define CFDH_AMG_OP_COL16 0x100
 int cfdh_get_amg_operator(cfdh_ctx *ctx, int hier, int level, int which, int64_t *nrow, int64_t *ncol, int64_t *nnz, int32_t *rowptr,
                           int32_t *col, double *vals);
 #define CFDH_AMG_VEC_DINV 0
```
